# OpenGene/gencore

Measured on AMD Instinct MI355X. Metric: consensus read-pairs/sec (whole node) + clustering HBM GB/s vs roofline, higher is better.
Workload: dtype u8

## Files before the change

### gencore_amd/capi.py

```python
import ctypes as C
import os

import numpy as np

GCE_ABI_VERSION = 3
GCE_NONE = 0xFFFFFFFF
GCE_MAX_SUPPORTING_READS = 100
UINT64_MAX = 0xFFFFFFFFFFFFFFFF

_HERE = os.path.dirname(os.path.abspath(__file__))
LIB_PATH = os.path.join(_HERE, "csrc", "libgencore_amd.so")

CORE_DTYPE = np.dtype(
    [("tid", "<i4"), ("pos", "<i4"), ("l_qname", "u1"), ("mapq", "u1"), ("bin", "<u2"), ("n_cigar", "<u2"),
     ("flag", "<u2"), ("l_qseq", "<i4"), ("mtid", "<i4"), ("mpos", "<i4"), ("isize", "<i4")])
assert CORE_DTYPE.itemsize == 32


class GceParams(C.Structure):
    _fields_ = [
        ("abi_version", C.c_int32), ("device", C.c_int32),
        ("proper_umi_diff_threshold", C.c_int32), ("unproper_umi_diff_threshold", C.c_int32),
        ("duplex_mismatch_threshold", C.c_int32), ("cluster_size_req", C.c_int32),
        ("base_score_req", C.c_int32), ("high_quality", C.c_int32), ("moderate_quality", C.c_int32),
        ("low_quality", C.c_int32), ("score_high", C.c_int32), ("score_moderate", C.c_int32),
        ("score_low", C.c_int32), ("score_bad", C.c_int32),
        ("skip_low_complexity_cluster_threshold", C.c_int32), ("duplex_only", C.c_int32),
        ("disable_duplex", C.c_int32), ("flush_period", C.c_int32),
        ("score_percent_req", C.c_double), ("umi_prefix", C.c_char * 32),
        ("n_targets", C.c_int32), ("target_len", C.c_void_p),
        ("tick_offset", C.c_int64), ("trailing_flush", C.c_int32), ("max_contig", C.c_int32),
    ]


class GceBatch(C.Structure):
    _fields_ = [
        ("n_reads", C.c_int64), ("core", C.c_void_p),
        ("qname_off", C.c_void_p), ("qname", C.c_void_p),
        ("cigar_off", C.c_void_p), ("cigar", C.c_void_p),
        ("seq_off", C.c_void_p), ("seq", C.c_void_p),
        ("qual_off", C.c_void_p), ("qual", C.c_void_p),
        ("nm", C.c_void_p), ("nm_type", C.c_void_p),
        ("mi_off", C.c_void_p), ("mi", C.c_void_p),
        ("qname_bytes", C.c_size_t), ("cigar_words", C.c_size_t), ("seq_bytes", C.c_size_t),
        ("qual_bytes", C.c_size_t), ("mi_bytes", C.c_size_t),
        ("tick", C.c_void_p),
    ]


class GceStats(C.Structure):
    _fields_ = [(n, C.c_int64) for n in (
        "reads", "bases", "reads_unmapped", "bases_unmapped", "base_mismatches", "reads_with_mismatches",
        "clusters", "multi_molecule_clusters", "molecules", "molecules_se", "molecules_pe", "sscs", "dcs",
        "uncounted_supporting_reads")] + [("supporting_hist", C.c_int64 * GCE_MAX_SUPPORTING_READS)]

    def as_dict(self):
        d = {n: int(getattr(self, n)) for n, _ in self._fields_[:-1]}
        d["supporting_hist"] = [int(x) for x in self.supporting_hist]
        return d

    def as_array(self):
        return np.frombuffer(bytes(self), dtype=np.int64).copy()


GCE_STATS_WORDS = 14 + GCE_MAX_SUPPORTING_READS
assert C.sizeof(GceStats) == 8 * GCE_STATS_WORDS


class GceResult(C.Structure):
    _fields_ = [
        ("n_reads", C.c_int64), ("n_out", C.c_int64), ("src", C.c_void_p), ("kind", C.c_void_p), ("qname_src", C.c_void_p),
        ("nm_new", C.c_void_p), ("fr", C.c_void_p), ("rr", C.c_void_p), ("mate", C.c_void_p), ("seq_off", C.c_void_p),
        ("qual_off", C.c_void_p), ("seq", C.c_void_p), ("qual", C.c_void_p), ("seq_bytes", C.c_size_t), ("qual_bytes", C.c_size_t),
        ("pre", GceStats), ("post", GceStats),
    ]


class GceTiming(C.Structure):
    _fields_ = [(n, C.c_double) for n in (
        "total_ms", "describe_ms", "cluster_ms", "csr_ms", "pairing_ms", "score_ms", "consensus_ms", "finish_ms", "output_ms")] + [
        ("n_clusters", C.c_int64), ("n_groups", C.c_int64), ("n_pairs", C.c_int64), ("n_leaders", C.c_int64)]

    def as_dict(self):
        return {n: getattr(self, n) for n, _ in self._fields_}


STATUS_NAMES = {
    0: "GCE_OK", -1: "GCE_ERR_INVALID", -2: "GCE_ERR_NO_DEVICE", -3: "GCE_ERR_HIP", -4: "GCE_ERR_OOM",
    -10: "GCE_ERR_UNSORTED", -11: "GCE_ERR_UMI_MISMATCH", -12: "GCE_ERR_NM_MISSING", -13: "GCE_ERR_UMI_PARSE",
    -14: "GCE_ERR_QNAME_SHORT", -15: "GCE_ERR_REF_WINDOW"}

EXPORTED_SYMBOLS = [
    "gce_params_default", "gce_detect_umi_prefix", "gce_create", "gce_destroy", "gce_set_reference", "gce_set_reference_ascii", "gce_set_reference_window",
    "gce_pack_reference", "gce_set_flush_events", "gce_submit", "gce_submit_device", "gce_process", "gce_drain", "gce_result_device",
    "gce_get_timing", "gce_get_vote_counters", "gce_get_consensus_counters", "gce_get_skipped_groups", "gce_get_index_counters", "gce_get_pairing_tiers", "gce_reset", "gce_last_error", "gce_status_message", "gce_abi_version",
    "gce_reserve", "gce_submit_async", "gce_submit_wait",
    "gce_bam_open", "gce_bam_close", "gce_bam_error", "gce_bam_get_info", "gce_bam_chunk", "gce_bam_write", "gce_bam_from_batch", "gce_sam_to_bam", "gce_bam_to_sam",
    "gce_fasta_load", "gce_fasta_get", "gce_fasta_free", "gce_run_bam", "gce_run_bam_hostcodec", "gce_run_bam_sharded", "gce_run_bam_sharded_hostcodec", "gce_raw_deflate_output", "gce_raw_read_deflated_async", "gce_bgzf_deflate", "gce_raw_deflate_output_codes", "gce_bgzf_deflate_codes", "gce_raw_attach_mirror", "gce_raw_select_shard", "gce_raw_merge_outputs", "gce_raw_begin", "gce_raw_push", "gce_raw_push_bgzf", "gce_bgzf_inflate", "gce_raw_finish", "gce_raw_build_output", "gce_raw_read_output_async", "gce_host_alloc", "gce_host_free", "gce_depth_stats", "gce_stats_payload_device", "gce_stats_payload_sum", "gce_stats_payload_read", "gce_run_bam_depth", "gce_depth_run_free", "gce_stats_device", "gce_stream_context", "gce_plan_shards", "gce_free", "gce_bed_load", "gce_bed_free",
    "gce_report_json", "gce_report_summary", "gce_bam_read_header", "gce_bam_header_free", "gce_run_bam_passes", "gce_device_bytes", "gce_bam_index", "gce_bam_sort", "gce_bam_sort_passes", "gce_sam_parse", "gce_sam_sort",
    "gce_sam_format", "gce_raw_format_output", "gce_raw_read_text_async", "gce_get_sam_format_counters",
    "gce_bam_calmd"]


class GceBamInfo(C.Structure):
    _fields_ = [("n_targets", C.c_int32), ("target_len", C.POINTER(C.c_uint32)), ("target_name", C.POINTER(C.c_char_p)),
                ("text", C.c_void_p), ("l_text", C.c_int64), ("n_records", C.c_int64),
                ("qname_bytes", C.c_uint64), ("cigar_words", C.c_uint64), ("seq_bytes", C.c_uint64), ("qual_bytes", C.c_uint64),
                ("mi_bytes", C.c_uint64), ("read_s", C.c_double), ("inflate_s", C.c_double), ("index_s", C.c_double)]


class GceDepth(C.Structure):
    _fields_ = [("n_targets", C.c_int32), ("bin_off", C.POINTER(C.c_int64)), ("pre_depth", C.POINTER(C.c_int64)), ("post_depth", C.POINTER(C.c_int64)),
                ("n_regions", C.c_int32), ("pre_bed", C.POINTER(C.c_int64)), ("post_bed", C.POINTER(C.c_int64))]


class GcePayloadLayout(C.Structure):
    _fields_ = [("stats_words", C.c_int32), ("n_targets", C.c_int32), ("n_bins", C.c_int64), ("n_regions", C.c_int32), ("total_words", C.c_int64),
                ("bin_off", C.POINTER(C.c_int64))]


class GceDepthRun(C.Structure):
    _fields_ = [("n_targets", C.c_int32), ("n_bins", C.c_int64), ("bin_off", C.POINTER(C.c_int64)), ("pre_depth", C.POINTER(C.c_int64)), ("post_depth", C.POINTER(C.c_int64)),
                ("n_regions", C.c_int32), ("region_tid", C.POINTER(C.c_int32)), ("region_start", C.POINTER(C.c_int32)), ("region_end", C.POINTER(C.c_int32)),
                ("pre_bed", C.POINTER(C.c_int64)), ("post_bed", C.POINTER(C.c_int64)), ("pre", GceStats), ("post", GceStats), ("payload_bytes", C.c_int64)]


class GcePassRun(C.Structure):
    _fields_ = [("n_passes", C.c_int32), ("single_pass", C.c_int32), ("reads_per_pass", C.c_int64 * 64), ("held_max", C.c_int64), ("peak_device_bytes", C.c_int64),
                ("budget_bytes", C.c_int64),
                ("fixed_bytes", C.c_int64), ("pass_room", C.c_int64), ("total_weight", C.c_int64), ("key_pass_s", C.c_double), ("pass_s", C.c_double * 64)]


class GceBaiRun(C.Structure):
    _fields_ = [("n_records", C.c_int64), ("n_no_coor", C.c_int64), ("n_bins", C.c_int64), ("n_chunks", C.c_int64), ("n_intervals", C.c_int64),
                ("n_ref", C.c_int32), ("pad", C.c_int32), ("read_s", C.c_double), ("gpu_s", C.c_double), ("write_s", C.c_double), ("total_s", C.c_double)]


class GceSortRun(C.Structure):
    _fields_ = [("n_records", C.c_int64), ("n_no_coor", C.c_int64), ("n_descents", C.c_int64), ("inflated_bytes", C.c_int64), ("out_bytes", C.c_int64),
                ("peak_device_bytes", C.c_int64), ("n_ref", C.c_int32), ("pad", C.c_int32), ("read_s", C.c_double), ("inflate_index_s", C.c_double),
                ("sort_s", C.c_double), ("gather_s", C.c_double), ("write_s", C.c_double), ("total_s", C.c_double)]


class GceCalmdRun(C.Structure):
    _fields_ = [("n_records", C.c_int64), ("n_rewritten", C.c_int64), ("n_unchanged", C.c_int64), ("n_no_ref", C.c_int64), ("n_nm_changed", C.c_int64),
                ("n_md_changed", C.c_int64), ("inflated_bytes", C.c_int64), ("out_record_bytes", C.c_int64), ("out_bytes", C.c_int64), ("peak_device_bytes", C.c_int64),
                ("n_ref", C.c_int32), ("pad", C.c_int32), ("read_s", C.c_double), ("inflate_index_s", C.c_double), ("calmd_s", C.c_double), ("write_s", C.c_double),
                ("total_s", C.c_double)]


class GceSortPassRun(C.Structure):
    _fields_ = [("n_passes", C.c_int32), ("in_core", C.c_int32), ("pass_bytes", C.c_int64), ("resident_bytes", C.c_int64), ("key_pass_s", C.c_double),
                ("plan_s", C.c_double), ("pass_s", C.c_double * 64)]


class GceBamRun(C.Structure):
    _fields_ = [("n_reads", C.c_int64), ("n_out", C.c_int64), ("open_s", C.c_double), ("read_s", C.c_double), ("inflate_s", C.c_double), ("index_s", C.c_double), ("submit_s", C.c_double),
                ("process_s", C.c_double), ("kernel_ms", C.c_double), ("drain_s", C.c_double), ("write_s", C.c_double),
                ("total_s", C.c_double), ("pre", GceStats), ("post", GceStats), ("peak_rss_kb", C.c_int64), ("rss_start_kb", C.c_int64), ("rss_end_kb", C.c_int64)]


class GceError(RuntimeError):
    def __init__(self, status, detail=""):
        self.status = status
        super().__init__("%s (%d): %s" % (STATUS_NAMES.get(status, "?"), status, detail))


_lib = None


def load_library(path=None, mode=C.RTLD_GLOBAL):
    global _lib
    if _lib is not None and path is None:
        return _lib
    p = path or os.environ.get("GCE_LIB") or LIB_PATH
    if not os.path.exists(p):
        raise OSError("libgencore_amd.so not built at %s — run `python -c 'import __graft_entry__ as g; g.build()'`" % p)
    lib = C.CDLL(p, mode=mode)
    lib.gce_params_default.argtypes = [C.POINTER(GceParams)]
    lib.gce_params_default.restype = None
    lib.gce_detect_umi_prefix.argtypes = [C.c_char_p, C.c_char * 32]
    lib.gce_detect_umi_prefix.restype = None
    lib.gce_create.argtypes = [C.POINTER(GceParams), C.POINTER(C.c_void_p)]
    lib.gce_destroy.argtypes = [C.c_void_p]
    lib.gce_destroy.restype = None
    lib.gce_set_reference.argtypes = [C.c_void_p, C.c_int32, C.c_void_p, C.c_int64]
    lib.gce_set_reference_ascii.argtypes = [C.c_void_p, C.c_int32, C.c_void_p, C.c_int64]
    lib.gce_set_reference_window.argtypes = [C.c_void_p, C.c_int32, C.c_int64, C.c_int64, C.c_void_p, C.c_int64]
    lib.gce_pack_reference.argtypes = [C.c_char_p, C.c_int64, C.c_void_p]
    lib.gce_pack_reference.restype = None
    lib.gce_set_flush_events.argtypes = [C.c_void_p, C.c_int32, C.c_void_p, C.c_void_p]
    lib.gce_submit.argtypes = [C.c_void_p, C.POINTER(GceBatch)]
    lib.gce_submit_device.argtypes = [C.c_void_p, C.POINTER(GceBatch)]
    lib.gce_process.argtypes = [C.c_void_p]
    lib.gce_drain.argtypes = [C.c_void_p, C.POINTER(GceResult)]
    lib.gce_result_device.argtypes = [C.c_void_p, C.POINTER(GceResult)]
    lib.gce_get_timing.argtypes = [C.c_void_p, C.POINTER(GceTiming)]
    lib.gce_get_vote_counters.argtypes = [C.c_void_p, C.POINTER(C.c_int64)]
    lib.gce_get_consensus_counters.argtypes = [C.c_void_p, C.POINTER(C.c_int64)]
    lib.gce_get_skipped_groups.argtypes = [C.c_void_p, C.POINTER(C.c_int64)]
    lib.gce_get_index_counters.argtypes = [C.c_void_p, C.POINTER(C.c_int64)]
    lib.gce_get_pairing_tiers.argtypes = [C.c_void_p, C.c_int64, C.c_void_p, C.c_void_p, C.POINTER(C.c_int64), C.POINTER(C.c_int64)]
    lib.gce_stats_device.argtypes = [C.c_void_p, C.POINTER(C.c_void_p)]
    lib.gce_stream_context.argtypes = [C.c_int32, C.c_void_p, C.c_int64, C.c_int32, C.c_void_p, C.POINTER(C.c_int32), C.POINTER(C.POINTER(C.c_int32)), C.POINTER(C.POINTER(C.c_int32))]
    lib.gce_plan_shards.argtypes = [C.c_int32, C.c_void_p, C.c_int64, C.c_int32, C.c_int32, C.c_void_p]
    lib.gce_free.argtypes = [C.c_void_p]
    lib.gce_free.restype = None
    lib.gce_reset.argtypes = [C.c_void_p]
    lib.gce_last_error.argtypes = [C.c_void_p]
    lib.gce_last_error.restype = C.c_char_p
    lib.gce_status_message.argtypes = [C.c_int]
    lib.gce_status_message.restype = C.c_char_p
    lib.gce_abi_version.restype = C.c_int
    lib.gce_reserve.argtypes = [C.c_void_p, C.c_int64, C.c_size_t, C.c_size_t, C.c_size_t, C.c_size_t]
    lib.gce_submit_async.argtypes = [C.c_void_p, C.POINTER(GceBatch), C.POINTER(C.c_int32)]
    lib.gce_submit_wait.argtypes = [C.c_void_p, C.c_int32]
    lib.gce_bam_open.argtypes = [C.c_char_p, C.c_int, C.POINTER(C.c_void_p)]
    lib.gce_bam_close.argtypes = [C.c_void_p]
    lib.gce_bam_close.restype = None
    lib.gce_bam_error.argtypes = [C.c_void_p]
    lib.gce_bam_error.restype = C.c_char_p
    lib.gce_bam_get_info.argtypes = [C.c_void_p, C.POINTER(GceBamInfo)]
    lib.gce_bam_chunk.argtypes = [C.c_void_p, C.c_int64, C.c_int64, C.c_int, C.POINTER(GceBatch)]
    lib.gce_bam_write.argtypes = [C.c_char_p, C.c_void_p, C.POINTER(GceResult), C.c_int, C.c_int]
    lib.gce_bam_from_batch.argtypes = [C.c_char_p, C.POINTER(GceBatch), C.c_int32, C.c_void_p, C.POINTER(C.c_char_p), C.c_char_p, C.c_int, C.c_int]
    lib.gce_sam_to_bam.argtypes = [C.c_char_p, C.c_char_p, C.c_int, C.c_int, C.c_char_p]
    lib.gce_bam_to_sam.argtypes = [C.c_char_p, C.c_char_p, C.c_int, C.c_char_p]
    lib.gce_fasta_load.argtypes = [C.c_char_p, C.c_int, C.POINTER(C.c_void_p)]
    lib.gce_fasta_get.argtypes = [C.c_void_p, C.POINTER(C.c_int32), C.POINTER(C.POINTER(C.c_char_p)), C.POINTER(C.POINTER(C.c_void_p)), C.POINTER(C.POINTER(C.c_int64))]
    lib.gce_fasta_free.argtypes = [C.c_void_p]
    lib.gce_fasta_free.restype = None
    lib.gce_depth_stats.argtypes = [C.c_void_p, C.c_int32, C.c_int32, C.c_void_p, C.c_void_p, C.c_void_p, C.POINTER(GceDepth)]
    lib.gce_stats_payload_device.argtypes = [C.c_void_p, C.c_int32, C.c_int32, C.c_void_p, C.c_void_p, C.c_void_p, C.POINTER(C.c_void_p), C.POINTER(GcePayloadLayout)]
    lib.gce_stats_payload_sum.argtypes = [C.POINTER(C.c_void_p), C.c_int32, C.POINTER(C.c_void_p), C.POINTER(GcePayloadLayout)]
    lib.gce_stats_payload_read.argtypes = [C.c_void_p, C.c_void_p, C.c_int64, C.c_void_p]
    lib.gce_run_bam_depth.argtypes = [C.c_char_p, C.c_char_p, C.c_char_p, C.c_char_p, C.c_int32, C.POINTER(GceParams), C.c_int32, C.c_void_p, C.c_int32, C.c_int, C.c_int,
                                      C.POINTER(GceBamRun), C.POINTER(GceDepthRun), C.c_char_p]
    lib.gce_run_bam_passes.argtypes = [C.c_char_p, C.c_char_p, C.c_char_p, C.c_char_p, C.c_int32, C.POINTER(GceParams), C.c_int32, C.c_int, C.c_int, C.c_size_t, C.c_int32, C.c_size_t,
                                       C.POINTER(GceBamRun), C.POINTER(GceDepthRun), C.POINTER(GcePassRun), C.c_char_p]
    lib.gce_device_bytes.argtypes = [C.POINTER(C.c_int64), C.POINTER(C.c_int64), C.c_int32]
    lib.gce_bam_index.argtypes = [C.c_char_p, C.c_char_p, C.c_int32, C.c_int, C.c_uint64, C.POINTER(GceBaiRun), C.c_char_p]
    if hasattr(lib, "gce_bam_sort"):
        lib.gce_bam_sort.argtypes = [C.c_char_p, C.c_char_p, C.c_int32, C.c_int, C.c_int, C.c_uint64, C.c_size_t, C.POINTER(GceSortRun), C.c_char_p]
    if hasattr(lib, "gce_bam_sort_passes"):
        lib.gce_bam_sort_passes.argtypes = [C.c_char_p, C.c_char_p, C.c_int32, C.c_int, C.c_int, C.c_uint64, C.c_size_t, C.c_int32, C.POINTER(GceSortRun),
                                            C.POINTER(GceSortPassRun), C.c_char_p]
    if hasattr(lib, "gce_sam_parse"):
        lib.gce_sam_parse.argtypes = [C.c_int32, C.c_char_p, C.c_size_t, C.c_int32, C.POINTER(C.c_char_p), C.c_void_p, C.c_size_t, C.POINTER(C.c_size_t), C.POINTER(C.c_int64),
                                      C.POINTER(C.c_int64), C.POINTER(C.c_int64), C.c_char_p]
    if hasattr(lib, "gce_sam_sort"):
        lib.gce_sam_sort.argtypes = [C.c_char_p, C.c_char_p, C.c_int32, C.c_int, C.c_int, C.c_uint64, C.c_size_t, C.POINTER(GceSortRun), C.POINTER(C.c_int64), C.c_char_p]
    if hasattr(lib, "gce_sam_format"):
        lib.gce_sam_format.argtypes = [C.c_int32, C.c_void_p, C.c_size_t, C.c_int32, C.POINTER(C.c_char_p), C.c_void_p, C.c_size_t, C.POINTER(C.c_size_t), C.POINTER(C.c_int64),
                                       C.POINTER(C.c_int64), C.POINTER(C.c_int64), C.c_char_p]
        lib.gce_raw_format_output.argtypes = [C.c_void_p, C.c_int32, C.POINTER(C.c_char_p), C.POINTER(C.c_uint64)]
        lib.gce_raw_read_text_async.argtypes = [C.c_void_p, C.c_uint64, C.c_void_p, C.c_size_t, C.POINTER(C.c_int32)]
        lib.gce_get_sam_format_counters.argtypes = [C.POINTER(C.c_int64)]
    if hasattr(lib, "gce_bam_calmd"):
        lib.gce_bam_calmd.argtypes = [C.c_char_p, C.c_char_p, C.c_char_p, C.c_int32, C.c_int, C.c_int, C.c_uint64, C.c_size_t, C.POINTER(GceCalmdRun), C.c_char_p]
    lib.gce_depth_run_free.argtypes = [C.POINTER(GceDepthRun)]
    lib.gce_depth_run_free.restype = None
    lib.gce_bed_load.argtypes = [C.c_char_p, C.c_int32, C.POINTER(C.c_char_p), C.POINTER(C.c_int32), C.POINTER(C.POINTER(C.c_int32)), C.POINTER(C.POINTER(C.c_int32)),
                                 C.POINTER(C.POINTER(C.c_int32)), C.POINTER(C.POINTER(C.c_char_p))]
    lib.gce_bed_free.argtypes = [C.c_int32, C.c_void_p, C.c_void_p, C.c_void_p, C.c_void_p]
    lib.gce_bed_free.restype = None
    lib.gce_report_json.argtypes = [C.c_char_p, C.POINTER(GceStats), C.POINTER(GceStats), C.POINTER(GceDepthRun), C.POINTER(C.c_char_p), C.POINTER(C.c_char_p),
                                    C.c_int32, C.c_int32, C.c_char_p, C.c_char * 256]
    lib.gce_report_summary.argtypes = [C.POINTER(GceStats), C.c_int32, C.c_char_p, C.c_size_t, C.POINTER(C.c_size_t)]
    lib.gce_bam_read_header.argtypes = [C.c_char_p, C.POINTER(C.c_int32), C.POINTER(C.POINTER(C.c_char_p)), C.POINTER(C.POINTER(C.c_uint32)), C.c_char * 256]
    lib.gce_bam_header_free.argtypes = [C.c_int32, C.POINTER(C.c_char_p), C.POINTER(C.c_uint32)]
    lib.gce_bam_header_free.restype = None
    lib.gce_bgzf_inflate.argtypes = [C.c_int32, C.c_void_p, C.c_size_t, C.c_int32, C.c_void_p, C.c_void_p, C.c_void_p, C.c_void_p, C.POINTER(C.c_int32)]
    lib.gce_bgzf_deflate.argtypes = [C.c_int32, C.c_void_p, C.c_size_t, C.c_uint32, C.c_void_p, C.c_size_t, C.POINTER(C.c_size_t)]
    if hasattr(lib, "gce_bgzf_deflate_codes"):
        lib.gce_bgzf_deflate_codes.argtypes = [C.c_int32, C.c_void_p, C.c_size_t, C.c_uint32, C.c_int32, C.c_void_p, C.c_size_t, C.POINTER(C.c_size_t)]
        lib.gce_raw_deflate_output_codes.argtypes = [C.c_void_p, C.c_int32, C.POINTER(C.c_uint64)]
    lib.gce_run_bam_sharded.argtypes = [C.c_char_p, C.c_char_p, C.c_char_p, C.POINTER(GceParams), C.c_int32, C.POINTER(C.c_int32), C.c_int32, C.c_int, C.c_int, C.POINTER(GceBamRun), C.c_char * 256]
    lib.gce_run_bam.argtypes = [C.c_char_p, C.c_char_p, C.c_char_p, C.POINTER(GceParams), C.c_int, C.c_int64, C.c_int, C.POINTER(GceBamRun), C.c_char * 256]
    if path is None:
        _lib = lib
    return lib


def default_params(lib=None, **overrides):
    p = GceParams()
# ... 25 lines not shown
```

### gencore_amd/csrc/engine.hip

```cpp
#include <hip/hip_runtime.h>
#include <hip/hip_ext.h>
#include <cstdio>
#include <cstdlib>
#include <algorithm>
#include <cstring>
#include <ctime>
#include <string>
#include <vector>

#include "gce_kernels.hpp"
#include "gce_pair2.hpp"
#include "gce_vote.hpp"
#include "gce_deep.hpp"
#include "gce_output.hpp"
#include "gce_depth.hpp"
#include "gce_inflate.hpp"
#include "gce_deflate.hpp"

namespace {

static thread_local double t_alloc_s = 0.0; static thread_local long t_alloc_n = 0; static thread_local size_t t_alloc_bytes = 0;
static inline double mono_s() { struct timespec ts; clock_gettime(CLOCK_MONOTONIC, &ts); return (double)ts.tv_sec + 1e-9 * (double)ts.tv_nsec; }
long long g_dev_live = 0, g_dev_peak = 0;
static int64_t g_pass_idx_ctr[4] = {0, 0, 0, 0};
inline void dev_bytes_add(long long d) {
    const long long now = __atomic_add_fetch(&g_dev_live, d, __ATOMIC_RELAXED);
    long long pk = __atomic_load_n(&g_dev_peak, __ATOMIC_RELAXED);
    while (now > pk && !__atomic_compare_exchange_n(&g_dev_peak, &pk, now, true, __ATOMIC_RELAXED, __ATOMIC_RELAXED)) {}
}
struct DevBuf {
    void *p = nullptr; size_t cap = 0;
    static size_t padded(size_t bytes) { return bytes + bytes / 8 + 256; }
    hipError_t ensure(size_t bytes) { return bytes <= cap && p ? hipSuccess : take(padded(bytes)); }
    hipError_t take(size_t want) {
        const double t0 = mono_s();
        release();
        hipError_t e = hipMalloc(&p, want);
        if (e == hipSuccess) { cap = want; dev_bytes_add((long long)want); } else p = nullptr;
        t_alloc_s += mono_s() - t0; t_alloc_n++; t_alloc_bytes += want;
        return e;
    }
    void release() { if (p) { (void)hipFree(p); dev_bytes_add(-(long long)cap); } p = nullptr; cap = 0; }
    template <class T> T *as() const { return (T *)p; }
};
struct ScopedBuf : DevBuf { ~ScopedBuf() { release(); } };

enum { EV_START = 0, EV_CLUSTER, EV_CSR, EV_DESCRIBE, EV_PAIRING, EV_SCORE, EV_CONSENSUS, EV_FINISH, EV_OUTPUT, EV_COUNT };

}

#include "gce_devstream.hpp"

struct HostRaw {
    uint8_t *p = nullptr; size_t n = 0, cap = 0;
    ~HostRaw() { free(p); }
    void resize(size_t k) { if (k > cap) { free(p); p = (uint8_t *)malloc(k ? k : 1); cap = p ? k : 0; } n = p ? k : 0; }
    uint8_t *data() { return p; }
    size_t size() const { return n; }
    bool empty() const { return n == 0; }
};

struct gce_engine {
    gce_params prm{};
    bool vote_off_logged = false;
    std::vector<uint32_t> target_len;
    std::string err;
    hipStream_t stream = nullptr;
    hipEvent_t ev[EV_COUNT]{};
    std::vector<DevBuf> ref_buf; std::vector<const uint8_t *> ref_ptr; std::vector<int64_t> ref_len, ref_win; bool have_win = false;
    DevBuf d_ref_ptr, d_ref_len, d_ref_win, d_target_len, d_target_cum;
    std::vector<const uint8_t *> up_ref_ptr; std::vector<int64_t> up_ref_len, up_win; std::vector<uint32_t> up_tl; const void *up_dev[5]{}; bool up_valid = false;
    std::vector<gce_core> h_core; std::vector<uint64_t> h_qoff, h_coff, h_soff, h_loff, h_mioff;
    std::vector<char> h_qname, h_mi; std::vector<uint32_t> h_cigar; std::vector<uint8_t> h_seq, h_qual, h_nmt; std::vector<int32_t> h_nm; std::vector<uint64_t> h_tick;
    std::vector<int32_t> h_ev_tid, h_ev_pos;
    bool have_mi = false, have_tick = false, have_events = false, host_mode = false, device_mode = false, processed = false;
    bool reserved = false; hipStream_t up_stream = nullptr; std::vector<hipEvent_t> up_events;
    hipStream_t aux_stream = nullptr; hipEvent_t aux_ev[4]{};
    size_t rs_n = 0, rs_q = 0, rs_c = 0, rs_s = 0, rs_l = 0, st_n = 0, st_q = 0, st_c = 0, st_s = 0, st_l = 0, st_m = 0; bool dev_concat = false;
    gce_batch dev_batch{};
    DevBuf b_core, b_qoff, b_qname, b_coff, b_cigar, b_soff, b_seq, b_loff, b_qual, b_nm, b_nmt, b_mioff, b_mi, b_tick;
    DevBuf uinfo, rdesc, spatch, slot, score, out_flag, orec, out_index, nmx;
    DevBuf o_src, o_kind, o_qsrc, o_nm, o_fr, o_rr, o_mate, o_soff, o_qoff, o_seq, o_qual, o_key, o_rec, o_ksoff, o_kqoff, o_krow, o_rank64, o_part3, ref_ascii;
    int64_t n_out = 0; size_t out_seq_bytes = 0, out_qual_bytes = 0; int dev_error = 0; uint32_t dev_error_read = 0;
    DevBuf lrec, lout, bhdr, blk_base, ev_tid, ev_pos, ev_read, table, toff;
    DevBuf raw, rw_tmp, rw_ncig, rw_nmpos, rw_rsize, rw_roff, rw_body; RecIdx rw;
    size_t raw_n = 0; bool raw_mode = false; int64_t raw_records = 0; uint64_t raw_body_bytes = 0;
    int64_t idx_ctr[4] = {0, 0, 0, 0};
    DevBuf z_comp, z_dir, z_err; size_t z_n = 0; std::vector<InfDir> z_members;
    DevBuf zo_slots, zo_sizes, zo_off, zo_out; uint64_t zo_bytes = 0;
    DevBuf sf_text; uint64_t sf_bytes = 0; int64_t raw_body_nrec = -1;
    std::vector<gce_engine *> mirrors;
    DevBuf sh_tickall, sh_shard, sh_flag, sh_sel, sh_core, sh_qoff, sh_coff, sh_soff, sh_loff, sh_nm, sh_nmt, sh_mioff, sh_tick, sh_roff, sh_nmpos, sh_keys, sh_stage; int64_t shard_n = -1;
    bool shard_cut_done = false;
    bool tab_clean = false; const void *tab_clean_ptr = nullptr; size_t tab_clean_cap = 0;
    DevBuf cl_ikey, cl_start, cl_n, cl_npairs, cl_ngroups, cl_gbase, cl_nresult, cl_hasumi, cl_tier;
    DevBuf members, sorted, pl, pr, pu, pg, gpl, gpr, grp_begin, grp_n, gl_cluster, g_begin, g_np;
    DevBuf slow_args, deep_list, k64, slow_list, left_list, pf_flag, pf_list, pq_flag, pq_list, p16_flag, p16_list, pd_slab, gen_flag, gen_list, score_list, gw, vlive, vb_start, rp_left, rp_right, rp_merge, rp_rmerge, rp_umi, rp_umilen, rp_state, rp_supp, rp_nm, rp_qsl, rp_qsr, scan_part, si;
    StreamInfo h_si{};
    void *si_pin = nullptr, *si_pin_dev = nullptr; unsigned long long si_seq = 0;
    gce_timing timing{};
    int64_t n = 0, n_pre = 0;
    DevBuf dp_binoff, dp_regoff, dp_rs, dp_re, dp_pmax, dp_sorted, dp_depth, dp_bed, dp_where;
    std::vector<int64_t> h_binoff, h_depth_pre, h_depth_post, h_bed_pre, h_bed_post; int64_t payload_words = 0;
    std::vector<uint8_t> r_kind; HostRaw r_seq, r_qual; std::vector<uint32_t> r_src, r_qsrc, r_mate; std::vector<int32_t> r_nm; std::vector<int16_t> r_fr, r_rr;
    std::vector<uint64_t> r_soff, r_qoff;
};

static int fail(gce_engine *e, int code, const std::string &msg) { if (e) e->err = msg; return code; }
#define HIPCHK(call) do { hipError_t _e = (call); if (_e != hipSuccess) return fail(e, _e == hipErrorOutOfMemory ? GCE_ERR_OOM : GCE_ERR_HIP, std::string(#call) + ": " + hipGetErrorString(_e)); } while (0)

extern "C" {

int gce_abi_version(void) { return GCE_ABI_VERSION; }

void gce_params_default(gce_params *p) {
    memset(p, 0, sizeof *p);
    p->abi_version = GCE_ABI_VERSION;
    p->proper_umi_diff_threshold = 1; p->unproper_umi_diff_threshold = 0; p->duplex_mismatch_threshold = 2;
    p->cluster_size_req = 1; p->base_score_req = 6; p->high_quality = 30; p->moderate_quality = 20; p->low_quality = 15;
    p->score_high = 8; p->score_moderate = 6; p->score_low = 4; p->score_bad = 2;
    p->skip_low_complexity_cluster_threshold = 1000; p->flush_period = 10000; p->score_percent_req = 0.8;
}

void gce_detect_umi_prefix(const char *q, char out[32]) {
    memset(out, 0, 32);
    if (strstr(q, "umi_")) strcpy(out, "umi");
    else if (strstr(q, "UMI_")) strcpy(out, "UMI");
}

const char *gce_status_message(int s) {
    switch (s) {
    case GCE_OK: return "ok";
    case GCE_ERR_INVALID: return "invalid argument or call order";
    case GCE_ERR_NO_DEVICE: return "no HIP device available (this engine has no CPU fallback)";
    case GCE_ERR_HIP: return "HIP runtime error";
    case GCE_ERR_OOM: return "out of device memory";
    case GCE_ERR_UNSORTED: return "ERROR: the input is unsorted. Please sort the input first.";
    case GCE_ERR_UMI_MISMATCH: return "The UMI of a read pair should be identical";
    case GCE_ERR_NM_MISSING: return "NM tag missing on a consensus template whose mismatch count changed";
    case GCE_ERR_UMI_PARSE: return "UMI parse: substr start beyond the end of the read name";
    case GCE_ERR_QNAME_SHORT: return "copyQName ERROR: desitination qname is shorter";
    case GCE_ERR_REF_WINDOW: return "reference window: a clustered read lies outside the bases staged for its contig";
    default: return "unknown status";
    }
}

const char *gce_last_error(const gce_engine *e) { return e ? e->err.c_str() : "null engine"; }

int gce_create(const gce_params *params, gce_engine **out) {
    if (!params || !out || params->abi_version != GCE_ABI_VERSION) return GCE_ERR_INVALID;
    if (params->proper_umi_diff_threshold < 0 || params->unproper_umi_diff_threshold < 0 || params->flush_period < 0) return GCE_ERR_INVALID;
    int ndev = 0;
    if (hipGetDeviceCount(&ndev) != hipSuccess || ndev <= 0 || params->device >= ndev) return GCE_ERR_NO_DEVICE;
    gce_engine *e = new gce_engine();
    e->prm = *params;
    if (e->prm.flush_period == 0) e->prm.flush_period = 10000;
    if (params->n_targets > 0 && params->target_len) e->target_len.assign(params->target_len, params->target_len + params->n_targets);
    e->prm.target_len = nullptr;
    if (hipSetDevice(params->device) != hipSuccess || hipStreamCreate(&e->stream) != hipSuccess) { delete e; return GCE_ERR_HIP; }
    for (auto &v : e->ev) (void)hipEventCreate(&v);
    *out = e;
    return GCE_OK;
}

void gce_destroy(gce_engine *e) {
    if (!e) return;
    (void)hipSetDevice(e->prm.device);
    (void)hipStreamSynchronize(e->stream);
    DevBuf *all[] = {&e->d_ref_ptr, &e->d_ref_len, &e->d_ref_win, &e->d_target_len, &e->d_target_cum, &e->b_core, &e->b_qoff, &e->b_qname, &e->b_coff, &e->b_cigar, &e->b_soff,
                     &e->b_seq, &e->b_loff, &e->b_qual, &e->b_nm, &e->b_nmt, &e->b_mioff, &e->b_mi, &e->b_tick, &e->uinfo, &e->rdesc, &e->spatch,
                     &e->slot, &e->score, &e->out_flag, &e->orec, &e->out_index, &e->nmx, &e->o_src, &e->o_kind, &e->o_qsrc, &e->o_nm, &e->o_fr, &e->o_rr, &e->o_mate,
                     &e->o_key, &e->o_rec, &e->o_ksoff, &e->o_kqoff, &e->o_krow, &e->o_rank64, &e->o_part3, &e->o_soff, &e->o_qoff, &e->o_seq, &e->o_qual, &e->ref_ascii, &e->lrec, &e->lout, &e->bhdr,
                     &e->blk_base, &e->ev_tid, &e->ev_pos, &e->ev_read, &e->table, &e->toff, &e->cl_ikey, &e->cl_start, &e->cl_n,
                     &e->cl_npairs, &e->cl_ngroups, &e->cl_gbase, &e->cl_nresult, &e->cl_hasumi, &e->cl_tier, &e->members, &e->sorted, &e->pl, &e->pr, &e->pu,
                     &e->pg, &e->gpl, &e->gpr, &e->grp_begin, &e->grp_n, &e->gl_cluster, &e->g_begin, &e->g_np, &e->deep_list, &e->k64, &e->slow_list, &e->pf_flag, &e->pf_list, &e->pq_flag, &e->pq_list, &e->left_list, &e->slow_args, &e->pd_slab, &e->gen_flag, &e->gen_list, &e->score_list, &e->gw, &e->vlive, &e->vb_start, &e->rp_left, &e->rp_right, &e->rp_merge, &e->rp_rmerge,
                     &e->rp_umi, &e->rp_umilen, &e->rp_state, &e->rp_supp, &e->rp_nm, &e->rp_qsl, &e->rp_qsr, &e->scan_part, &e->si};
    for (auto *b : all) b->release();
    for (DevBuf *b : {&e->z_comp, &e->z_dir, &e->z_err, &e->raw, &e->rw_tmp, &e->rw_ncig, &e->rw_nmpos, &e->rw_rsize, &e->rw_roff, &e->rw_body, &e->sf_text}) b->release();
    e->rw.release();
    for (DevBuf *b : {&e->zo_slots, &e->zo_sizes, &e->zo_off, &e->zo_out, &e->p16_flag, &e->p16_list}) b->release();
    for (DevBuf *b : {&e->sh_tickall, &e->sh_shard, &e->sh_flag, &e->sh_sel, &e->sh_core, &e->sh_qoff, &e->sh_coff, &e->sh_soff, &e->sh_loff, &e->sh_nm, &e->sh_nmt, &e->sh_mioff, &e->sh_tick, &e->sh_roff, &e->sh_nmpos, &e->sh_keys, &e->sh_stage}) b->release();
    for (DevBuf *b : {&e->dp_binoff, &e->dp_regoff, &e->dp_rs, &e->dp_re, &e->dp_pmax, &e->dp_sorted, &e->dp_depth, &e->dp_bed, &e->dp_where}) b->release();
    for (auto ev : e->up_events) (void)hipEventDestroy(ev);
    if (e->up_stream) { (void)hipStreamSynchronize(e->up_stream); (void)hipStreamDestroy(e->up_stream); }
    if (e->aux_stream) { (void)hipStreamSynchronize(e->aux_stream); (void)hipStreamDestroy(e->aux_stream); }
    for (auto &v : e->aux_ev) if (v) (void)hipEventDestroy(v);
    for (auto &b : e->ref_buf) b.release();
    for (auto &v : e->ev) if (v) (void)hipEventDestroy(v);
    if (e->stream) (void)hipStreamDestroy(e->stream);
    if (e->si_pin) (void)hipHostFree(e->si_pin);
    delete e;
}

void gce_pack_reference(const char *bases, int64_t n, uint8_t *out) {
    memset(out, 0, (size_t)((n + 1) / 2));
    for (int64_t i = 0; i < n; i++) {
        uint8_t code;
        switch (bases[i]) { case 'A': code = 1; break; case 'T': code = 2; break; case 'C': code = 3; break; case 'G': code = 4; break; default: code = 0; }
        out[i >> 1] |= (i & 1) ? (uint8_t)(code << 4) : code;
    }
}

int gce_set_reference(gce_engine *e, int32_t tid, const uint8_t *nibbles, int64_t n_bases) {
    if (!e || tid < 0 || n_bases < 0) return GCE_ERR_INVALID;
    (void)hipSetDevice(e->prm.device);
    if ((size_t)tid >= e->ref_buf.size()) { e->ref_buf.resize(tid + 1); e->ref_ptr.resize(tid + 1, nullptr); e->ref_len.resize(tid + 1, 0); }
    if (!nibbles) { e->ref_ptr[tid] = nullptr; e->ref_len[tid] = 0; return GCE_OK; }
    size_t bytes = (size_t)((n_bases + 1) / 2);
    HIPCHK(e->ref_buf[tid].ensure(bytes + 16));
    hipPointerAttribute_t attr; bool is_dev = hipPointerGetAttributes(&attr, nibbles) == hipSuccess && attr.type == hipMemoryTypeDevice;
    (void)hipGetLastError();
    HIPCHK(hipMemcpyAsync(e->ref_buf[tid].p, nibbles, bytes, is_dev ? hipMemcpyDeviceToDevice : hipMemcpyHostToDevice, e->stream));
    HIPCHK(hipStreamSynchronize(e->stream));
    e->ref_ptr[tid] = e->ref_buf[tid].as<uint8_t>(); e->ref_len[tid] = n_bases;
    if (2 * (size_t)tid + 1 < e->ref_win.size()) e->ref_win[2 * tid] = e->ref_win[2 * tid + 1] = 0;
    return GCE_OK;
}

int gce_set_reference_ascii(gce_engine *e, int32_t tid, const char *bases, int64_t n_bases) {
    if (!e || tid < 0 || n_bases < 0 || (!bases && n_bases > 0)) return GCE_ERR_INVALID;
    (void)hipSetDevice(e->prm.device);
    if ((size_t)tid >= e->ref_buf.size()) { e->ref_buf.resize(tid + 1); e->ref_ptr.resize(tid + 1, nullptr); e->ref_len.resize(tid + 1, 0); }
    const size_t bytes = (size_t)((n_bases + 1) / 2);
    HIPCHK(e->ref_buf[tid].ensure(bytes + 16));
    HIPCHK(e->ref_ascii.ensure((size_t)n_bases + 16));
    hipPointerAttribute_t attr; const bool is_dev = hipPointerGetAttributes(&attr, bases) == hipSuccess && attr.type == hipMemoryTypeDevice;
    (void)hipGetLastError();
    if (n_bases) {
        HIPCHK(hipMemcpyAsync(e->ref_ascii.p, bases, (size_t)n_bases, is_dev ? hipMemcpyDeviceToDevice : hipMemcpyHostToDevice, e->stream));
        const unsigned grid = (unsigned)std::min<uint64_t>((bytes + 255) / 256, 65535u * 4u);
        hipLaunchKernelGGL(k_pack_reference, dim3(grid), dim3(256), 0, e->stream, (const char *)e->ref_ascii.p, n_bases, e->ref_buf[tid].as<uint8_t>());
    }
    HIPCHK(hipStreamSynchronize(e->stream));
    HIPCHK(hipGetLastError());
    e->ref_ptr[tid] = e->ref_buf[tid].as<uint8_t>(); e->ref_len[tid] = n_bases;
    if (2 * (size_t)tid + 1 < e->ref_win.size()) e->ref_win[2 * tid] = e->ref_win[2 * tid + 1] = 0;
    return GCE_OK;
}

int gce_set_reference_window(gce_engine *e, int32_t tid, int64_t contig_len, int64_t win_start, const char *bases, int64_t n_bases) {
    if (!e || tid < 0 || contig_len < 0 || win_start < 0 || (win_start & 1) || n_bases < 0 || win_start + n_bases > contig_len || (!bases && n_bases > 0)) return GCE_ERR_INVALID;
    const int rc = gce_set_reference_ascii(e, tid, bases, n_bases);
    if (rc != GCE_OK) return rc;
    if (e->ref_win.size() < 2 * e->ref_ptr.size()) e->ref_win.resize(2 * e->ref_ptr.size(), 0);
    e->ref_ptr[tid] = e->ref_buf[tid].as<uint8_t>() - (win_start >> 1);
    e->ref_len[tid] = contig_len;
    e->ref_win[2 * tid] = win_start; e->ref_win[2 * tid + 1] = win_start + n_bases;
    e->have_win = true;
    return GCE_OK;
}

int gce_reset(gce_engine *e) {
    if (!e) return GCE_ERR_INVALID;
    e->h_core.clear(); e->h_qoff.clear(); e->h_coff.clear(); e->h_soff.clear(); e->h_loff.clear(); e->h_mioff.clear(); e->h_tick.clear();
    e->h_qname.clear(); e->h_mi.clear(); e->h_cigar.clear(); e->h_seq.clear(); e->h_qual.clear(); e->h_nmt.clear(); e->h_nm.clear();
    e->have_mi = e->have_tick = e->host_mode = e->device_mode = e->processed = e->raw_mode = false; e->n = 0; e->n_out = 0; e->shard_n = -1; e->shard_cut_done = false;
    e->st_n = e->st_q = e->st_c = e->st_s = e->st_l = e->st_m = 0; e->dev_concat = false;
    return GCE_OK;
}

int gce_set_flush_events(gce_engine *e, int32_t n_events, const int32_t *ev_tid, const int32_t *ev_pos) {
    if (!e || n_events < 0 || (n_events > 0 && (!ev_tid || !ev_pos))) return GCE_ERR_INVALID;
    e->h_ev_tid.assign(ev_tid, ev_tid + n_events); e->h_ev_pos.assign(ev_pos, ev_pos + n_events);
// ... 396 lines not shown
    const bool same = e->up_valid && e->up_ref_ptr == e->ref_ptr && e->up_ref_len == e->ref_len && e->up_tl == e->target_len && e->up_win == win && memcmp(dev_now, e->up_dev, sizeof dev_now) == 0;
    if (!same) {
        e->up_valid = false;
        if (nref) {
            HIPCHK(hipMemcpyAsync(e->d_ref_ptr.p, e->ref_ptr.data(), (size_t)nref * 8, hipMemcpyHostToDevice, e->stream));
            HIPCHK(hipMemcpyAsync(e->d_ref_len.p, e->ref_len.data(), (size_t)nref * 8, hipMemcpyHostToDevice, e->stream));
        }
        std::vector<uint64_t> cum(e->target_len.size()); uint64_t acc = 0;
        for (size_t i = 0; i < cum.size(); i++) { cum[i] = acc; acc += e->target_len[i]; }
        if (!e->target_len.empty()) {
            HIPCHK(hipMemcpyAsync(e->d_target_len.p, e->target_len.data(), e->target_len.size() * 4, hipMemcpyHostToDevice, e->stream));
            HIPCHK(hipMemcpyAsync(e->d_target_cum.p, cum.data(), cum.size() * 8, hipMemcpyHostToDevice, e->stream));
        }
        if (!win.empty()) HIPCHK(hipMemcpyAsync(e->d_ref_win.p, win.data(), win.size() * 8, hipMemcpyHostToDevice, e->stream));
        HIPCHK(hipStreamSynchronize(e->stream));
        e->up_ref_ptr = e->ref_ptr; e->up_ref_len = e->ref_len; e->up_tl = e->target_len; e->up_win = win; memcpy(e->up_dev, dev_now, sizeof dev_now);
        e->up_valid = true;
    }
    DevParams p{};
    p.proper_thr = e->prm.proper_umi_diff_threshold; p.unproper_thr = e->prm.unproper_umi_diff_threshold;
    p.duplex_mismatch_thr = e->prm.duplex_mismatch_threshold; p.cluster_size_req = e->prm.cluster_size_req; p.base_score_req = e->prm.base_score_req;
    p.high_q = e->prm.high_quality; p.moderate_q = e->prm.moderate_quality; p.low_q = e->prm.low_quality;
    p.s_high = e->prm.score_high; p.s_moderate = e->prm.score_moderate; p.s_low = e->prm.score_low; p.s_bad = e->prm.score_bad;
    p.skip_low_complexity_thr = e->prm.skip_low_complexity_cluster_threshold; p.duplex_only = e->prm.duplex_only; p.disable_duplex = e->prm.disable_duplex;
    p.period = e->prm.flush_period; p.score_percent_req = e->prm.score_percent_req;
    {
        int mn = std::min(std::min(p.s_high, p.s_moderate), std::min(p.s_low, p.s_bad)), mx = std::max(std::max(p.s_high, p.s_moderate), std::max(p.s_low, p.s_bad));
        p.score_bias = std::max(0, 3 - mn); p.score_max = std::max(0, mx + 4);
        if (p.score_max + p.score_bias > 255) return fail(e, GCE_ERR_INVALID, "score constants out of range");
        auto by = [&](int sc) { return (uint32_t)((sc + p.score_bias) & 0xFF); };
        p.q2s_lut = by(p.s_bad) | by(p.s_low) << 8 | by(p.s_moderate) << 16 | by(p.s_high) << 24;
        p.thr_low4 = 0x01010101u * (uint32_t)(p.low_q & 0xFF); p.thr_mod4 = 0x01010101u * (uint32_t)(p.moderate_q & 0xFF); p.thr_high4 = 0x01010101u * (uint32_t)(p.high_q & 0xFF);
        p.q2s_swar_ok = p.low_q >= 0 && p.low_q <= p.moderate_q && p.moderate_q <= p.high_q && p.high_q <= 127;
        p.s_min_lb = mn;
        p.vote_ok = mn >= 0 && mx + 4 <= 120 && p.moderate_q >= 0 && p.moderate_q <= 127 && p.base_score_req <= 100 && p.q2s_swar_ok;
        p.vote_accept_by_qual = std::min(std::min(p.s_moderate, p.s_high), mn + 4) >= std::max(p.base_score_req, 1);
        if (!p.vote_ok && !e->vote_off_logged) {
            e->vote_off_logged = true;
            const char *why = !p.q2s_swar_ok ? "quality thresholds not nested (low <= moderate <= high <= 127)" : mn < 0 ? "a score constant below 0"
                            : mx + 4 > 120 ? "a score constant above 116" : (p.moderate_q < 0 || p.moderate_q > 127) ? "moderate quality outside 0..127" : "base_score_req above 100";
            fprintf(stderr, "gencore_amd: k_vote off for this engine (%s): every group goes to the per-side kernels\n", why);
        }
    }
    memcpy(p.prefix, e->prm.umi_prefix, 32); p.prefix[31] = 0; p.prefix_len = (int)strlen(p.prefix);
    p.n_targets = (int)e->target_len.size(); p.target_len = e->d_target_len.as<uint32_t>(); p.target_cum = e->target_len.empty() ? nullptr : e->d_target_cum.as<uint64_t>();
    p.tick_offset = e->have_tick ? 0 : e->prm.tick_offset; p.tick_epoch0 = p.tick_offset / p.period; p.tick_rem0 = (int32_t)(p.tick_offset % p.period); p.trailing_flush = e->have_tick ? 0 : e->prm.trailing_flush;
    {
        uint32_t mx = 1; for (uint32_t v : e->target_len) mx = std::max(mx, v);
        int bt = 1; while (bt < 31 && (1ll << bt) < (long long)std::max<size_t>(e->target_len.size(), 1)) bt++;
        int bl = 1; while (bl < 32 && (1ull << bl) <= (uint64_t)mx) bl++;
        p.key_bt = bt; p.key_bl = bl;
    }
    p.n_ref = nref; p.ref_data = e->d_ref_ptr.as<const uint8_t *>(); p.ref_len = e->d_ref_len.as<int64_t>(); p.ref_win = win.empty() ? nullptr : e->d_ref_win.as<int64_t>();

    Work w{};
    const int64_t n_sblk = (N + SB_READS - 1) / SB_READS;
    w.n_sblk = n_sblk;
    const int64_t max_events = e->have_tick ? (int64_t)e->h_ev_tid.size() + 2 : (p.tick_offset % p.period + N) / p.period + 2;
    w.max_events = (int)max_events;
    uint64_t T = ((uint64_t)n1 + (uint64_t)n1 / 4 + 2 * SCAN_TILE - 1) / SCAN_TILE * SCAN_TILE;
    w.tsize = T; w.tinv = 1.0 / (double)T;
    {
        uint64_t genome = 0; for (uint32_t v : e->target_len) genome += v;
        const uint64_t qmax = (genome * TAB_WAYS + TAB_WAYS) / T + 1;
        int cb = 1; while (cb < 33 && (1ull << cb) <= (uint64_t)N + 1024) cb++;
        int qb = 1; while (qb < 52 && (1ull << qb) <= qmax) qb++;
        p.nw_cb = cb; p.nw_bd = 62 - cb - qb; p.nw_ok = !e->target_len.empty() && p.nw_bd >= 1;
        if (p.nw_bd > 40) p.nw_bd = 40;
    }
    const size_t qual_bytes = hb.qual_bytes ? hb.qual_bytes : 1;
    const size_t nsb1 = (size_t)(n_sblk > 0 ? n_sblk : 1);
#define ENS(buf, bytes) HIPCHK(e->buf.ensure(bytes))
    ENS(uinfo, n1 * 8); ENS(rdesc, n1 * sizeof(ReadDescP)); ENS(spatch, n1 * 4); ENS(slot, n1 * 4 + 16); ENS(score, qual_bytes + 64);
    ENS(out_flag, n1 + 144);        ENS(nmx, n1 * 4); ENS(orec, n1 * sizeof(OutRec)); ENS(out_index, n1 * 4);
    ENS(lrec, nsb1 * SB_READS * sizeof(LeadRec)); ENS(lout, nsb1 * SB_READS * sizeof(LeadOut));
    ENS(bhdr, nsb1 * sizeof(BlkHdr)); ENS(blk_base, nsb1 * 4);
    ENS(ev_tid, (size_t)max_events * 4); ENS(ev_pos, (size_t)max_events * 4); ENS(ev_read, (size_t)max_events * 4);
    ENS(table, T * sizeof(TabEntry)); ENS(toff, T * 4);
    ENS(k64, n1 * 24); ENS(members, n1 * 4); ENS(sorted, n1 * 4); ENS(pl, n1 * 4); ENS(pr, n1 * 4); ENS(pu, n1 * 4); ENS(pg, n1 * 4); ENS(gpl, n1 * 4); ENS(gpr, n1 * 4);
    ENS(grp_begin, n1 * 4); ENS(grp_n, n1 * 4); ENS(slow_list, n1 * 4 + 64);
    w.slow_list = e->slow_list.as<uint32_t>();
    ENS(deep_list, (n1 / 64 + 64) * 16); w.deep_list = e->deep_list.p;
    const unsigned nblk_N = cdiv(n1, SCAN_TILE);
    ENS(scan_part, std::max<size_t>(2 * nsb1, (size_t)2 * nblk_N) * 8 + 16);     ENS(si, sizeof(StreamInfo));
    w.uinfo = e->uinfo.as<uint64_t>(); w.rdesc = e->rdesc.as<ReadDescP>(); w.spatch = e->spatch.as<uint32_t>();
    w.slot = e->slot.as<uint32_t>(); w.score = e->score.as<int8_t>();
    w.out_flag = e->out_flag.as<uint8_t>(); w.nmx = e->nmx.as<uint32_t>(); w.orec = e->orec.as<OutRec>(); w.out_index = e->out_index.as<uint32_t>();
    w.lrec = e->lrec.as<LeadRec>(); w.lout = e->lout.as<LeadOut>(); w.bhdr = e->bhdr.as<BlkHdr>(); w.blk_base = e->blk_base.as<uint32_t>();
    w.ev_tid = e->ev_tid.as<int32_t>(); w.ev_pos = e->ev_pos.as<int32_t>(); w.ev_read = e->ev_read.as<uint32_t>();
    w.tab = e->table.as<TabEntry>(); w.toff = e->toff.as<uint32_t>();
    w.k64 = e->k64.as<uint64_t>(); w.members = e->members.as<uint32_t>(); w.sorted = e->sorted.as<uint32_t>(); w.pl = e->pl.as<uint32_t>(); w.pr = e->pr.as<uint32_t>();
    w.pu = e->pu.as<uint32_t>(); w.pg = e->pg.as<uint32_t>(); w.gpl = e->gpl.as<uint32_t>(); w.gpr = e->gpr.as<uint32_t>();
    w.grp_begin = e->grp_begin.as<uint32_t>(); w.grp_n = e->grp_n.as<uint32_t>();
    w.scan_part = e->scan_part.as<uint64_t>(); w.si = e->si.as<StreamInfo>();
    ENS(cl_ikey, n1 * 4); ENS(cl_start, n1 * 4); ENS(cl_n, n1 * 4);
    w.cl_ikey = e->cl_ikey.as<uint32_t>(); w.cl_start = e->cl_start.as<uint32_t>(); w.cl_n = e->cl_n.as<uint32_t>();

    StreamInfo init{}; init.first_unmapped = NONE32; init.err_key = ~0ull; init.lq_min = 0x7FFFFFFF; init.lq_max = -1;
    if (e->have_tick) { init.n_events = init.n_events_a = (int)e->h_ev_tid.size(); }
    HIPCHK(hipMemcpyAsync(e->si.p, &init, sizeof init, hipMemcpyHostToDevice, e->stream));
    if (e->have_tick && !e->h_ev_tid.empty()) {
        HIPCHK(hipMemcpyAsync(e->ev_tid.p, e->h_ev_tid.data(), e->h_ev_tid.size() * 4, hipMemcpyHostToDevice, e->stream));
        HIPCHK(hipMemcpyAsync(e->ev_pos.p, e->h_ev_pos.data(), e->h_ev_pos.size() * 4, hipMemcpyHostToDevice, e->stream));
    }
    hipStream_t s = e->stream;
    if (!e->tab_clean || e->tab_clean_ptr != e->table.p || e->tab_clean_cap != e->table.cap) {
        HIPCHK(hipMemsetAsync(e->table.p, 0, e->table.cap, s));
        e->tab_clean_ptr = e->table.p; e->tab_clean_cap = e->table.cap;
    }
    e->tab_clean = false;
    HIPCHK(hipEventRecord(e->ev[EV_START], s));
    HIPCHK(hipMemsetAsync(e->out_flag.p, 0, n1, s));
    if (N > 0) LAUNCH_EV(k_cluster, dim3((unsigned)n_sblk), dim3(SB_T), s, e->ev[EV_CLUSTER], b, p, w);
#ifdef CL_PROF
    if (N > 0) {
        StreamInfo hs; (void)hipStreamSynchronize(s); (void)hipMemcpy(&hs, e->si.p, sizeof hs, hipMemcpyDeviceToHost);
        static const char *nm[3] = {"key records + keys", "LDS leaders", "stores"};
        const double blocks = (double)hs.prof[15];
        fprintf(stderr, "k_cluster phases, mean per block (us), %.0f blocks:", blocks);
        for (int k = 0; k < 3; k++) fprintf(stderr, " %s %.2f;", nm[k], blocks ? hs.prof[k] / blocks / 100.0 : 0.0);
        fprintf(stderr, "\n");
    }
#endif
    if (N <= 0) HIPCHK(hipEventRecord(e->ev[EV_CLUSTER], s));
    CANARY("EV_CLUSTER");
    if (N > 0) {
        if (!e->have_tick) {
            hipLaunchKernelGGL(k_blk_scan, dim3(1), dim3(1024), 0, s, w, p);
            hipLaunchKernelGGL(k_events, dim3(cdiv(max_events, EV_T / 64)), dim3(EV_T), 0, s, b, p, w);
        }
        const unsigned nb4 = cdiv(n_sblk, 4);
        hipLaunchKernelGGL(k_leaders, dim3(nb4), dim3(256), 0, s, b, p, w);
        hipLaunchKernelGGL(k_num_reduce, dim3(nb4), dim3(256), 0, s, w, p.nw_cb);
        hipLaunchKernelGGL(k_scan_partials, dim3(1), dim3(1024), 0, s, w.scan_part, (uint64_t)nb4, &w.si->n_clusters, (unsigned long long *)nullptr);
        hipLaunchKernelGGL(k_num_apply, dim3(nb4), dim3(256), 0, s, w);
        LAUNCH_EV(k_scatter, dim3((unsigned)n_sblk), dim3(SB_T), s, e->ev[EV_CSR], N, w);
    } else HIPCHK(hipEventRecord(e->ev[EV_CSR], s));
    CANARY("EV_CSR");
    unsigned long long si_seq1 = 0;
    if ((rc = read_si_begin(e, &si_seq1)) != GCE_OK) return rc;
    if (N > 0) {
#ifndef GCE_DESCRIBE_BLOCKS
#define GCE_DESCRIBE_BLOCKS 32768
#endif
        const int64_t n_tiles = (N + 255) / 256;
        int tpb = (int)((n_tiles + GCE_DESCRIBE_BLOCKS - 1) / GCE_DESCRIBE_BLOCKS); if (tpb < 1) tpb = 1;
        LAUNCH_EV(k_describe, dim3(cdiv(n_tiles, tpb)), dim3(256), s, e->ev[EV_DESCRIBE], b, p, w, tpb);
    } else HIPCHK(hipEventRecord(e->ev[EV_DESCRIBE], s));
    CANARY("EV_DESCRIBE");
    if ((rc = read_si_end(e, si_seq1)) != GCE_OK) return rc;
    HIPCHK(hipGetLastError());
    e->tab_clean = true;
    const uint32_t C = (uint32_t)e->h_si.n_clusters;
    const size_t c1 = C ? C : 1;
    ENS(cl_npairs, c1 * 4); ENS(cl_ngroups, c1 * 4); ENS(cl_gbase, c1 * 4); ENS(cl_nresult, c1 * 4); ENS(cl_hasumi, c1); ENS(cl_tier, c1);
    w.cl_npairs = e->cl_npairs.as<uint32_t>(); w.cl_ngroups = e->cl_ngroups.as<uint32_t>(); w.cl_gbase = e->cl_gbase.as<uint32_t>();
    w.cl_nresult = e->cl_nresult.as<uint32_t>(); w.cl_hasumi = e->cl_hasumi.as<uint8_t>(); w.cl_tier = e->cl_tier.as<uint8_t>();
    uint32_t NG = 0;
    bool si_behind_describe = false;
    if (C > 0 && e->dev_error == 0) {
        ENS(left_list, c1 * 4 + 64); w.left_list = e->left_list.as<uint32_t>();
        ENS(pf_flag, c1 + 64); ENS(pf_list, c1 * 4); ENS(pq_flag, c1 + 64); ENS(pq_list, c1 * 4); ENS(p16_flag, c1 + 64); ENS(p16_list, c1 * 4);
        w.pf_flag = e->pf_flag.as<uint8_t>(); w.pf_list = e->pf_list.as<uint32_t>(); w.pq_flag = e->pq_flag.as<uint8_t>(); w.pq_list = e->pq_list.as<uint32_t>(); w.p16_flag = e->p16_flag.as<uint8_t>(); w.p16_list = e->p16_list.as<uint32_t>();
        const bool pair_classes = (double)N > 10.0 * (double)C;
        if (!pair_classes) fill_many(s, {FillSeg{e->pf_flag.p, c1, 0u, 0u}, FillSeg{e->pq_flag.p, c1, 0u, 0u}});
        const unsigned nbc = cdiv(C, SCAN_TILE);
        auto compact = [&](uint8_t *flag, uint32_t *list, unsigned long long *count) {
            hipLaunchKernelGGL(k_flag_reduce, dim3(nbc), dim3(256), 0, s, (const uint8_t *)flag, (uint64_t)C, w.scan_part);
            hipLaunchKernelGGL(k_scan_partials, dim3(1), dim3(1024), 0, s, w.scan_part, (uint64_t)nbc, count, (unsigned long long *)nullptr);
            hipLaunchKernelGGL(k_flag_apply, dim3(nbc), dim3(256), 0, s, (const uint8_t *)flag, (uint64_t)C, (const uint64_t *)w.scan_part, list);
        };
#ifdef PS_STOP
        {
            hipEvent_t a_, b_, c_; (void)hipEventCreate(&a_); (void)hipEventCreate(&b_); (void)hipEventCreate(&c_);
            (void)hipEventRecord(a_, s);
            hipLaunchKernelGGL(k_pairing_sub<16>, dim3(cdiv(C, 4 * WAVES_PER_BLOCK)), dim3(256), 0, s, b, p, w, C, (const uint32_t *)nullptr, (const unsigned long long *)nullptr, w.pq_flag, 0);
            (void)hipEventRecord(b_, s);
            hipLaunchKernelGGL(k_pairing_sub<32>, dim3(cdiv(C, 2 * WAVES_PER_BLOCK)), dim3(256), 0, s, b, p, w, C, (const uint32_t *)nullptr, (const unsigned long long *)nullptr, w.pf_flag, 0);
            (void)hipEventRecord(c_, s); (void)hipEventSynchronize(c_);
            float m1 = 0, m2 = 0; (void)hipEventElapsedTime(&m1, a_, b_); (void)hipEventElapsedTime(&m2, b_, c_);
            fprintf(stderr, "k_pairing_sub up to tick %d: <16> %.3f ms, <32> over ALL clusters %.3f ms\n", PS_STOP, m1, m2);
            return fail(e, GCE_ERR_INVALID, "experiment build");
        }
#endif
        ENS(pd_slab, PD_BIG_BLOCKS * PD_SLAB);
        if (pair_classes) {
            hipLaunchKernelGGL(k_pair_class_reduce, dim3(nbc), dim3(256), 0, s, (const uint32_t *)w.cl_n, C, w.scan_part);
            hipLaunchKernelGGL(k_scan_partials, dim3(1), dim3(1024), 0, s, w.scan_part, (uint64_t)nbc, &w.si->n_p16_items, &w.si->n_pq_items);
            hipLaunchKernelGGL(k_pair_class_apply, dim3(nbc), dim3(256), 0, s, (const uint32_t *)w.cl_n, C, (const uint64_t *)w.scan_part, w.p16_list, w.pq_list, w.pf_list, w.si);
            static const bool tiers_aux = getenv("GCE_NO_AUX_STREAM") == nullptr;
            hipStream_t s2 = s;
            if (tiers_aux) {
                if ((rc = aux_ready(e)) != GCE_OK) return rc;
                s2 = e->aux_stream;
                HIPCHK(hipEventRecord(e->aux_ev[0], s));
                HIPCHK(hipStreamWaitEvent(s2, e->aux_ev[0], 0));
            }
            hipLaunchKernelGGL(k_pairing_fast, dim3(2048), dim3(256), 0, s2, b, p, w, C, (const uint32_t *)w.pf_list);
            hipLaunchKernelGGL(k_pairing_deep<false>, dim3(256), dim3(PD_T), 0, s2, b, p, w, (uint8_t *)nullptr);
            if (tiers_aux) HIPCHK(hipEventRecord(e->aux_ev[1], s2));
            hipLaunchKernelGGL(k_pairing_sub<16>, dim3(cdiv(C, 4 * WAVES_PER_BLOCK)), dim3(256), 0, s, b, p, w, C, (const uint32_t *)w.p16_list, (const unsigned long long *)&w.si->n_p16_items, w.pq_flag, 1);
            hipLaunchKernelGGL(k_pairing_sub<32>, dim3(cdiv(C, 2 * WAVES_PER_BLOCK)), dim3(256), 0, s, b, p, w, C, (const uint32_t *)w.pq_list, (const unsigned long long *)&w.si->n_pq_items, w.pf_flag, 1);
            if (tiers_aux) HIPCHK(hipStreamWaitEvent(s, e->aux_ev[1], 0));
        } else {
            hipLaunchKernelGGL(k_pairing_sub<16>, dim3(cdiv(C, 4 * WAVES_PER_BLOCK)), dim3(256), 0, s, b, p, w, C, (const uint32_t *)nullptr, (const unsigned long long *)nullptr, w.pq_flag, 0);
            compact(w.pq_flag, w.pq_list, &w.si->n_pq_items);
            hipLaunchKernelGGL(k_pairing_sub<32>, dim3(cdiv(C, 2 * WAVES_PER_BLOCK)), dim3(256), 0, s, b, p, w, C, (const uint32_t *)w.pq_list, (const unsigned long long *)&w.si->n_pq_items, w.pf_flag, 0);
            compact(w.pf_flag, w.pf_list, &w.si->n_pf_items);
            hipLaunchKernelGGL(k_pairing_fast, dim3(2048), dim3(256), 0, s, b, p, w, C, (const uint32_t *)w.pf_list);
            hipLaunchKernelGGL(k_pairing_deep<false>, dim3(256), dim3(PD_T), 0, s, b, p, w, (uint8_t *)nullptr);
        }
        hipLaunchKernelGGL(k_pairing_deep<true>, dim3(PD_BIG_BLOCKS), dim3(PD_T), 0, s, b, p, w, e->pd_slab.as<uint8_t>());
        hipLaunchKernelGGL(k_pairing_slow<0>, dim3(1024), dim3(256), 0, s, b, p, w);
        hipLaunchKernelGGL(k_pairing_slow<1>, dim3(1024, 16), dim3(256), 0, s, b, p, w);
        hipLaunchKernelGGL(k_pairing_slow<2>, dim3(1024), dim3(256), 0, s, b, p, w);
        const unsigned nblk_C = cdiv(C, SCAN_TILE);
        hipLaunchKernelGGL(k_scan_reduce, dim3(nblk_C), dim3(256), 0, s, (const uint32_t *)w.cl_ngroups, (uint64_t)C, w.scan_part);
        hipLaunchKernelGGL(k_scan_partials, dim3(1), dim3(1024), 0, s, w.scan_part, (uint64_t)nblk_C, &w.si->n_pairs , &w.si->n_groups);
        hipLaunchKernelGGL(k_u32_apply, dim3(nblk_C), dim3(256), 0, s, (const uint32_t *)w.cl_ngroups, w.cl_gbase, (uint64_t)C, (const uint64_t *)w.scan_part);
        ENS(gl_cluster, n1 * 4); ENS(g_begin, n1 * 4); ENS(g_np, n1 * 4); ENS(gw, n1 * 8); ENS(vlive, n1 * 16);
        const size_t vb_cap = ((VB_MINW + 3) * n1) / VB_W + 8;
        ENS(vb_start, vb_cap * 4);
        w.gl_cluster = e->gl_cluster.as<uint32_t>(); w.g_begin = e->g_begin.as<uint32_t>(); w.g_np = e->g_np.as<uint32_t>();
        w.gw = e->gw.as<uint64_t>(); w.vlive = e->vlive.as<uint4>(); w.vb_start = e->vb_start.as<uint32_t>();
        HIPCHK(hipMemsetAsync(e->vb_start.p, 0xFF, vb_cap * 4, s));
        hipLaunchKernelGGL(k_group_fill, dim3(cdiv(C, 256)), dim3(256), 0, s, p, w, C, (uint32_t)VB_W, (uint32_t)VB_MINW);
        hipLaunchKernelGGL(k_u64_reduce, dim3(nblk_N), dim3(256), 0, s, (const uint64_t *)w.gw, (const unsigned long long *)&w.si->n_groups, w.scan_part);
        hipLaunchKernelGGL(k_u64_partials, dim3(1), dim3(1024), 0, s, w.scan_part, (const unsigned long long *)&w.si->n_groups, &w.si->vote_weight, &w.si->n_live);
        LAUNCH_EV(k_vote_batches, dim3(nblk_N), dim3(256), s, e->ev[EV_PAIRING], w, (const unsigned long long *)&w.si->n_groups, (const uint64_t *)w.scan_part);
        CANARY("EV_PAIRING");
        if ((rc = read_si(e)) != GCE_OK) return rc;
        HIPCHK(hipGetLastError());
        si_behind_describe = true;
        NG = (uint32_t)e->h_si.n_groups;
    } else HIPCHK(hipEventRecord(e->ev[EV_PAIRING], s));
    const size_t g1 = NG ? NG : 1;
    ENS(gen_list, g1 * 8); ENS(gen_flag, g1 * 2 + 64); ENS(score_list, n1 * 4 + 64);       ENS(rp_left, g1 * 4); ENS(rp_right, g1 * 4); ENS(rp_merge, g1 * 4); ENS(rp_rmerge, g1 * 4); ENS(rp_umi, g1 * 8);
    ENS(rp_umilen, g1 * 2); ENS(rp_state, g1); ENS(rp_supp, g1 * 4); ENS(rp_nm, g1 * 8); ENS(rp_qsl, g1 * 4); ENS(rp_qsr, g1 * 4);
    w.gen_list = e->gen_list.as<uint32_t>(); w.gen_flag = e->gen_flag.as<uint8_t>(); w.score_list = e->score_list.as<uint32_t>();
    w.rp_left = e->rp_left.as<uint32_t>(); w.rp_right = e->rp_right.as<uint32_t>();
    w.rp_merge = e->rp_merge.as<uint32_t>(); w.rp_rmerge = e->rp_rmerge.as<uint32_t>(); w.rp_umi = e->rp_umi.as<const char *>();
    w.rp_umilen = e->rp_umilen.as<uint16_t>(); w.rp_state = e->rp_state.as<uint8_t>(); w.rp_supp = e->rp_supp.as<int32_t>();
    w.rp_nm = e->rp_nm.as<int32_t>(); w.rp_qsl = e->rp_qsl.as<uint32_t>(); w.rp_qsr = e->rp_qsr.as<uint32_t>();
    if (NG > 0 && e->dev_error == 0) {
        {
            SlowArgs sa; sa.b = b; sa.p = p; sa.w = w;
            HIPCHK(e->slow_args.ensure(sizeof sa));
            HIPCHK(hipMemcpyAsync(e->slow_args.p, &sa, sizeof sa, hipMemcpyHostToDevice, s));
        }
        fill_many(s, {FillSeg{e->gen_flag.p, g1 * 2, 0u, 0u},
                      FillSeg{e->rp_nm.p, g1 * 8, 0xFFu, 0u},
                      FillSeg{e->rp_left.p, g1 * 4, 0xFFu, 0u}, FillSeg{e->rp_right.p, g1 * 4, 0xFFu, 0u}});
        const uint32_t n_live = (uint32_t)e->h_si.n_live;
#ifdef VB_XCD
        const unsigned nbatch = (((unsigned)(e->h_si.vote_weight / VB_W) + 1u) + 7u) & ~7u;
#else
        const unsigned nbatch = (unsigned)(e->h_si.vote_weight / VB_W) + 1u;
#endif
#ifdef VB_STOP
        {
            hipEvent_t a_, b_; (void)hipEventCreate(&a_); (void)hipEventCreate(&b_);
            (void)hipEventRecord(a_, s); hipLaunchKernelGGL(k_vote, dim3(nbatch), dim3(VB_T), 0, s, b, p, w, n_live); (void)hipEventRecord(b_, s); (void)hipEventSynchronize(b_);
            float ms_ = 0; (void)hipEventElapsedTime(&ms_, a_, b_); fprintf(stderr, "k_vote up to tick %d: %.3f ms\n", VB_STOP, ms_);
            return fail(e, GCE_ERR_INVALID, "experiment build");
        }
#endif
        LAUNCH_EV(k_vote, dim3(nbatch), dim3(VB_T), s, e->ev[EV_SCORE], b, p, w, n_live);
        CANARY("EV_SCORE");
        const bool deep_stream = ((double)N > 48.0 * (double)NG || getenv("GCE_FORCE_AUX_STREAM")) && !getenv("GCE_NO_AUX_STREAM");
        const unsigned cf_cap = deep_stream ? 32768u : 4096u, sc2_cap = deep_stream ? 16384u : 2048u;
        const unsigned cf_grid = std::min<unsigned>(cdiv(2ull * NG, WAVES_PER_BLOCK), cf_cap);
        const unsigned sc2_grid = std::min<unsigned>(cdiv(N, 2 * WAVES_PER_BLOCK * 64), sc2_cap);
        if (deep_stream) {
            if ((rc = aux_ready(e)) != GCE_OK) return rc;
            HIPCHK(hipEventRecord(e->aux_ev[0], s));
            HIPCHK(hipStreamWaitEvent(e->aux_stream, e->aux_ev[0], 0));
            hipLaunchKernelGGL(k_score2, dim3(sc2_grid), dim3(256), 0, e->aux_stream, b, p, w);
            HIPCHK(hipEventRecord(e->aux_ev[1], e->aux_stream));
            hipLaunchKernelGGL(k_deep_prepare, dim3(1024), dim3(256), 0, s, b, p, w);
            HIPCHK(hipStreamWaitEvent(s, e->aux_ev[1], 0));
            hipLaunchKernelGGL(k_consensus_fast, dim3(cf_grid), dim3(256), 0, s, b, p, w);
        } else {
            hipLaunchKernelGGL(k_score2, dim3(sc2_grid), dim3(256), 0, s, b, p, w);
            hipLaunchKernelGGL(k_deep_prepare, dim3(1024), dim3(256), 0, s, b, p, w);
            hipLaunchKernelGGL(k_consensus_fast, dim3(cf_grid), dim3(256), 0, s, b, p, w);
        }
        hipLaunchKernelGGL(k_vote_deep, dim3(1024), dim3(DV_T), 0, s, b, p, w);
        LAUNCH_EV(k_consensus_slow, dim3(512), dim3(256), s, e->ev[EV_CONSENSUS], (const SlowArgs *)e->slow_args.p);
        CANARY("EV_CONSENSUS");
        hipLaunchKernelGGL(k_group_tail, dim3(cdiv(NG, 256)), dim3(256), 0, s, b, p, w, NG);
        if (!p.disable_duplex) {
            const unsigned nbc = cdiv(C, SCAN_TILE);
// ... 193 lines not shown
    HIPCHK(e->dp_depth.ensure((size_t)words * 8 + 64)); HIPCHK(e->dp_bed.ensure((size_t)nreg * 16 + 64));
    HIPCHK(hipMemsetAsync(e->dp_depth.p, 0, (size_t)words * 8, s)); HIPCHK(hipMemsetAsync(e->dp_bed.p, 0, (size_t)nreg * 16 + 16, s));
    DepthCtx c; c.bin_off = e->dp_binoff.as<int64_t>(); c.n_targets = nt; c.step = step; c.reg_off = e->dp_regoff.as<int32_t>();
    c.r_start = e->dp_rs.as<int32_t>(); c.r_end = e->dp_re.as<int32_t>(); c.r_pmax = e->dp_pmax.as<int32_t>(); c.contig_sorted = e->dp_sorted.as<uint8_t>();
    long long *pay = e->dp_depth.as<long long>();
    unsigned long long *dpre = (unsigned long long *)pay + 2 * GCE_STATS_WORDS, *dpost = dpre + nbins, *bpre = e->dp_bed.as<unsigned long long>(), *bpost = bpre + nreg;
    const uint64_t n = (uint64_t)e->n_pre, no = (uint64_t)e->n_out;
    if (n) hipLaunchKernelGGL(k_depth, dim3(cdiv(n, DP_T * DP_RPT)), dim3(DP_T), 0, s, e->dev_batch.core, (const uint32_t *)nullptr, n, c, dpre, bpre);
    if (no) hipLaunchKernelGGL(k_depth, dim3(cdiv(no, DP_T * DP_RPT)), dim3(DP_T), 0, s, e->dev_batch.core, (const uint32_t *)e->o_src.p, no, c, dpost, bpost);
    const int fin = std::max(2 * GCE_STATS_WORDS, (int)n_regions);
    hipLaunchKernelGGL(k_payload_finish, dim3(cdiv(fin, 256)), dim3(256), 0, s, (const StreamInfo *)e->si.p, (const int32_t *)e->dp_where.p, n_regions, (const unsigned long long *)e->dp_bed.p, nreg, pay, nbins);
    HIPCHK(hipGetLastError());
    HIPCHK(hipStreamSynchronize(s));
    layout->stats_words = 2 * GCE_STATS_WORDS; layout->n_targets = nt; layout->n_bins = nbins; layout->n_regions = n_regions; layout->total_words = words; layout->bin_off = e->h_binoff.data();
    e->payload_words = words;
    *payload = (const int64_t *)pay;
    return GCE_OK;
}

int gce_stats_payload_read(gce_engine *e, const int64_t *payload, int64_t n_words, int64_t *host) {
    if (!e || !payload || !host || n_words < 0) return GCE_ERR_INVALID;
    (void)hipSetDevice(e->prm.device);
    if (n_words) HIPCHK(hipMemcpyAsync(host, payload, (size_t)n_words * 8, hipMemcpyDeviceToHost, e->stream));
    HIPCHK(hipStreamSynchronize(e->stream));
    return GCE_OK;
}

int gce_depth_stats(gce_engine *e, int32_t step, int32_t n_regions, const int32_t *r_tid, const int32_t *r_start, const int32_t *r_end, gce_depth *out) {
    if (!e || !out) return GCE_ERR_INVALID;
    const int64_t *pay = nullptr; gce_payload_layout lay;
    int rc = gce_stats_payload_device(e, step, n_regions, r_tid, r_start, r_end, &pay, &lay);
    if (rc != GCE_OK) return rc;
    hipStream_t s = e->stream;
    const int64_t nbins = lay.n_bins;
    e->h_depth_pre.resize(nbins); e->h_depth_post.resize(nbins); e->h_bed_pre.assign(n_regions, 0); e->h_bed_post.assign(n_regions, 0);
    const int64_t *d0 = pay + lay.stats_words;
    if (nbins) { HIPCHK(hipMemcpyAsync(e->h_depth_pre.data(), d0, nbins * 8, hipMemcpyDeviceToHost, s)); HIPCHK(hipMemcpyAsync(e->h_depth_post.data(), d0 + nbins, nbins * 8, hipMemcpyDeviceToHost, s)); }
    if (n_regions) { HIPCHK(hipMemcpyAsync(e->h_bed_pre.data(), d0 + 2 * nbins, (size_t)n_regions * 8, hipMemcpyDeviceToHost, s)); HIPCHK(hipMemcpyAsync(e->h_bed_post.data(), d0 + 2 * nbins + n_regions, (size_t)n_regions * 8, hipMemcpyDeviceToHost, s)); }
    HIPCHK(hipStreamSynchronize(s));
    out->n_targets = lay.n_targets; out->bin_off = e->h_binoff.data(); out->pre_depth = e->h_depth_pre.data(); out->post_depth = e->h_depth_post.data();
    out->n_regions = n_regions; out->pre_bed = e->h_bed_pre.data(); out->post_bed = e->h_bed_post.data();
    return GCE_OK;
}

int gce_stats_device(gce_engine *e, const int64_t **pre_then_post) {
    if (!e || !pre_then_post || !e->processed || e->dev_error) return GCE_ERR_INVALID;
    *pre_then_post = (const int64_t *)e->si.as<StreamInfo>()->pre;
    return GCE_OK;
}

int gce_get_timing(gce_engine *e, gce_timing *out) {
    if (!e || !out) return GCE_ERR_INVALID;
    *out = e->timing;
    return GCE_OK;
}

int gce_get_vote_counters(gce_engine *e, int64_t out[4]) {
    if (!e || !out || !e->processed) return GCE_ERR_INVALID;
    out[0] = (int64_t)e->h_si.vote_rounds2; out[1] = (int64_t)e->h_si.vote_rounds2_unaligned;
    out[2] = (int64_t)(e->h_si.hand_on >> 32); out[3] = (int64_t)e->h_si.n_groups;
    return GCE_OK;
}

int gce_get_consensus_counters(gce_engine *e, int64_t out[5]) {
    if (!e || !out || !e->processed) return GCE_ERR_INVALID;
    out[0] = 2 * (int64_t)(e->h_si.n_groups ? e->h_si.n_live : 0) - (int64_t)(e->h_si.hand_on >> 32);
    out[1] = (int64_t)e->h_si.cs_fast; out[2] = (int64_t)e->h_si.cs_prep; out[3] = (int64_t)e->h_si.cs_deep; out[4] = (int64_t)e->h_si.cs_slow;
    return GCE_OK;
}

int gce_get_skipped_groups(gce_engine *e, int64_t out[2]) {
    if (!e || !out || !e->processed) return GCE_ERR_INVALID;
    out[0] = e->h_si.n_groups ? (int64_t)e->h_si.n_groups - (int64_t)e->h_si.n_live : 0;
    out[1] = e->h_si.n_groups ? (int64_t)(e->h_si.vote_weight / VB_W) + 1 : 0;
    return GCE_OK;
}

int gce_get_index_counters(gce_engine *e, int64_t out[4]) {
    if (!out) return GCE_ERR_INVALID;
    for (int k = 0; k < 4; k++) out[k] = e ? e->idx_ctr[k] : __atomic_load_n(&g_pass_idx_ctr[k], __ATOMIC_RELAXED);
    return GCE_OK;
}

int gce_get_pairing_tiers(gce_engine *e, int64_t cap, uint8_t *tier, uint32_t *read, int64_t *n_clusters, int64_t counts[GCE_PAIR_TIERS]) {
    if (!e || !e->processed || e->dev_error || cap < 0) return GCE_ERR_INVALID;
    const int64_t C = (int64_t)e->h_si.n_clusters;
    if (n_clusters) *n_clusters = C;
    if (counts) for (int k = 0; k < GCE_PAIR_TIERS; k++) counts[k] = 0;
    if (C == 0) return GCE_OK;
    if (!e->cl_tier.p || e->cl_tier.cap < (size_t)C) return fail(e, GCE_ERR_INVALID, "no pairing ran in the last gce_process");
    (void)hipSetDevice(e->prm.device);
    std::vector<uint8_t> t((size_t)C);
    HIPCHK(hipMemcpy(t.data(), e->cl_tier.p, (size_t)C, hipMemcpyDeviceToHost));
    if (counts) for (int64_t c = 0; c < C; c++) { if (t[c] >= GCE_PAIR_TIERS) return fail(e, GCE_ERR_INVALID, "a cluster has no pairing tier"); counts[t[c]]++; }
    const int64_t m = C < cap ? C : cap;
    if (tier) memcpy(tier, t.data(), (size_t)m);
    if (read && m > 0) {
        std::vector<uint32_t> st((size_t)m), pl((size_t)(e->n > 0 ? e->n : 1));
        HIPCHK(hipMemcpy(st.data(), e->cl_start.p, (size_t)m * 4, hipMemcpyDeviceToHost));
        HIPCHK(hipMemcpy(pl.data(), e->gpl.p, pl.size() * 4, hipMemcpyDeviceToHost));
        for (int64_t c = 0; c < m; c++) read[c] = (t[c] == GCE_PAIR_TIER_NEVER || st[c] >= pl.size()) ? 0xFFFFFFFFu : pl[st[c]];
    }
    return GCE_OK;
}

}

#include "gce_plan.hpp"
#include "gce_bamdev.hpp"
#include "gce_passes.hpp"
#include "gce_bai.hpp"
#include "gce_samdev.hpp"
#include "gce_samfmt.hpp"
#undef MCHK
#include "gce_sort.hpp"
#include "gce_calmd.hpp"
```

### gencore_amd/csrc/gce_device.hpp

```cpp
#pragma once
#include <hip/hip_runtime.h>
#include <stdint.h>
#include "../../include/gencore_amd.h"

#define GCE_WAVE 64
#define NONE32 0xFFFFFFFFu
#define EMPTY64 0xFFFFFFFFFFFFFFFFull

enum : uint32_t { THR_PROPER = 0, THR_UNPROPER = 1, THR_NEVER = 2, THR_RAW = 3 };
enum : uint8_t { TIER_NEVER = 0, TIER_SUB16 = 1, TIER_SUB32 = 2, TIER_FAST = 3, TIER_DEEP_LDS = 4, TIER_DEEP_DEVICE = 5, TIER_GENERIC = 6 };
enum : uint8_t { CLS_DROP = 0, CLS_CLUSTERED = 1, CLS_BYPASS = 2 };

struct DevBatch {
    int64_t n;
    const gce_core *core;
    const uint64_t *qname_off; const char *qname;
    const uint64_t *cigar_off; const uint32_t *cigar;
    const uint64_t *seq_off;   uint8_t *seq;
    const uint64_t *qual_off;  uint8_t *qual;
    const int32_t *nm; const uint8_t *nm_type;
    const uint64_t *mi_off; const char *mi;
    const uint64_t *tick;
};

struct DevParams {
    int32_t proper_thr, unproper_thr, duplex_mismatch_thr, cluster_size_req, base_score_req;
    int32_t high_q, moderate_q, low_q;
    int32_t s_high, s_moderate, s_low, s_bad;
    int32_t skip_low_complexity_thr, duplex_only, disable_duplex, period;
    int32_t score_bias, score_max;
    uint32_t q2s_lut;
    uint32_t thr_low4, thr_mod4, thr_high4;
    int32_t q2s_swar_ok;
    double score_percent_req;
    char prefix[32];
    int32_t prefix_len;
    int32_t n_targets;
    const uint32_t *target_len;
    const uint64_t *target_cum;
    int32_t key_bt, key_bl;
    int32_t nw_ok, nw_cb, nw_bd;
    int32_t vote_ok, vote_accept_by_qual, s_min_lb;
    int64_t tick_offset;
    int64_t tick_epoch0; int32_t tick_rem0;
    int32_t trailing_flush;
    int32_t n_ref;
    const uint8_t *const *ref_data;
    const int64_t *ref_len;
    const int64_t *ref_win;
};

#define GCE_PRE_SLOTS 64
struct StreamInfo {
    unsigned long long n_clustered;
    unsigned int first_unmapped;
    unsigned long long err_key;
    int n_events;
    int n_events_a;
    unsigned int n_slow;
    unsigned long long prof[32];
    unsigned int n_deep;
    unsigned long long hand_on;
    unsigned int n_slow_pair;
    unsigned int n_slow_pair2;
    unsigned int pair_next, pair_next2;
    unsigned int prep_next, deep_next;
    int lq_min, lq_max;
    unsigned long long n_clusters, n_groups, n_pairs, n_out;
    unsigned long long n_pairs_total;
    unsigned long long vote_weight;
    unsigned long long n_live;
    unsigned long long n_leaders;
    unsigned long long out_units;
    unsigned long long n_pf_items;
    unsigned long long n_pq_items;
    unsigned long long n_p16_items;
    unsigned long long vote_rounds2;
    unsigned long long vote_rounds2_unaligned;
    unsigned int n_raw;
    unsigned int cs_fast, cs_prep, cs_deep, cs_slow;
    long long pre[GCE_STATS_WORDS];
    long long post[GCE_STATS_WORDS];
    long long post_slot[GCE_PRE_SLOTS][8];
    long long pre_slot[GCE_PRE_SLOTS][8];
};

__device__ __forceinline__ void raise_error(StreamInfo *si, int code, uint32_t read) {
    atomicMin(&si->err_key, ((unsigned long long)read << 8) | (unsigned long long)((-code) & 0xFF));
}

__device__ __forceinline__ int lane_id() { return threadIdx.x & 63; }

__device__ __forceinline__ int cig_op(uint32_t w) { return (int)(w & 0xF); }
__device__ __forceinline__ int cig_len(uint32_t w) { return (int)(w >> 4); }
__device__ __forceinline__ int consumes_query(int op) { return (0x193 >> op) & 1; }
__device__ __forceinline__ int consumes_ref(int op) { return (0x18D >> op) & 1; }

struct __attribute__((aligned(16))) ReadDescP {
    uint32_t so_lo, qo_lo;
    uint32_t c0;
    uint32_t pos_fl;
    uint16_t lq, mo, ml, nc;
    int32_t tid;
    uint32_t hi;
};
static_assert(sizeof(ReadDescP) == 32, "ReadDescP must stay 32 bytes");
struct ReadDesc {
    uint64_t so, qo;
    uint32_t c0;
    int32_t pos, lq, isize;
    int32_t mo, ml;
    int32_t tid;
    uint16_t nc, lastm;
    int32_t rlen;
};
#define RLEN_WALK (-0x40000000)
__device__ __forceinline__ void store_desc(ReadDescP *base, uint64_t i, uint64_t so, uint64_t qo, uint32_t c0, int32_t pos, bool isize_nz, int lq, int mo, int ml, int nc, int32_t tid, uint32_t last_op) {
    union { ReadDescP d; uint4 q[2]; } u;
    u.d.so_lo = (uint32_t)so; u.d.qo_lo = (uint32_t)qo; const uint32_t lastm = cig_op(last_op) == 0 ? min((uint32_t)cig_len(last_op), 65535u) : 0u;
    u.d.hi = ((uint32_t)(so >> 32) & 0xFFu) | ((uint32_t)(qo >> 32) & 0xFFu) << 8 | lastm << 16;
    u.d.c0 = c0; u.d.pos_fl = (uint32_t)pos | (isize_nz ? 0x80000000u : 0u);
    u.d.lq = (uint16_t)lq; u.d.mo = (uint16_t)mo; u.d.ml = (uint16_t)ml; u.d.nc = (uint16_t)nc; u.d.tid = tid;
    uint4 *dst = reinterpret_cast<uint4 *>(base + i); dst[0] = u.q[0]; dst[1] = u.q[1];
}
__device__ __forceinline__ ReadDesc load_desc(const ReadDescP *base, uint32_t i) {
    union { ReadDescP d; uint4 q[2]; } u;
    const uint4 *src = reinterpret_cast<const uint4 *>(base + i);
    u.q[0] = src[0]; u.q[1] = src[1];
    ReadDesc r;
    r.so = (uint64_t)u.d.so_lo | (uint64_t)(u.d.hi & 0xFFu) << 32; r.qo = (uint64_t)u.d.qo_lo | (uint64_t)((u.d.hi >> 8) & 0xFFu) << 32;
    r.c0 = u.d.c0; r.pos = (int32_t)(u.d.pos_fl & 0x7FFFFFFFu); r.isize = (int32_t)(u.d.pos_fl >> 31);
    r.lq = u.d.lq; r.mo = u.d.mo; r.ml = u.d.ml; r.nc = u.d.nc; r.tid = u.d.tid; r.lastm = (uint16_t)(u.d.hi >> 16);
    r.rlen = u.d.nc == 1 ? (int32_t)(cig_len(u.d.c0) * consumes_ref(cig_op(u.d.c0))) : (u.d.nc == 0 ? 0 : RLEN_WALK);
    return r;
}


__device__ inline bool d_is_part_of(const uint32_t *part, int np, const uint32_t *whole, int nw, bool left) {
    if (nw < np) return false;
    for (int i = 0; i < np; i++) {
        uint32_t a = left ? part[i] : part[np - 1 - i];
        uint32_t b = left ? whole[i] : whole[nw - 1 - i];
        if (cig_op(a) != cig_op(b)) return false;
        int la = cig_len(a), lb = cig_len(b);
        if (la > lb) return false;
        if (la < lb && i != np - 1) {
            if (i != np - 2) return false;
            uint32_t nx = left ? part[i + 1] : part[np - 2 - i];
            if (cig_op(nx) != 5 ) return false;
        }
    }
    return true;
}

__device__ inline int d_ref_offset(const uint32_t *cig, int n, int qpos) {
    int ref = 0, query = 0;
    for (int i = 0; i < n; i++) {
        int op = cig_op(cig[i]), len = cig_len(cig[i]);
        int cq = consumes_query(op), cr = consumes_ref(op);
// ... 305 lines not shown
```

### gencore_amd/csrc/gce_kernels.hpp

```cpp
#pragma once
#include "gce_device.hpp"

#define CHUNK 256
#define WAVES_PER_BLOCK 4

struct __attribute__((aligned(16))) OutRec { uint32_t qname_src, mate; int16_t nm_new, fr, rr; uint16_t pad; };
static_assert(sizeof(OutRec) == 16, "OutRec must stay 16 bytes");

struct Work {
    uint64_t *uinfo;
    ReadDescP *rdesc;
    uint32_t *spatch;
    uint32_t *slot;
    int8_t *score;
    uint8_t *out_flag; OutRec *orec;
    uint32_t *nmx;
    uint32_t *out_index;
    struct LeadRec *lrec; struct LeadOut *lout;
    struct BlkHdr *bhdr; uint32_t *blk_base; int64_t n_sblk;
    int32_t *ev_tid, *ev_pos; uint32_t *ev_read; int max_events;
    struct TabEntry *tab; uint32_t *toff; uint64_t tsize; double tinv;
    uint32_t *cl_ikey, *cl_start, *cl_n, *cl_npairs, *cl_ngroups, *cl_gbase, *cl_nresult; uint8_t *cl_hasumi;
    uint8_t *cl_tier;
    uint32_t *members, *sorted, *pl, *pr, *pu, *pg, *gpl, *gpr, *grp_begin, *grp_n;
    uint64_t *k64;
    uint32_t *gl_cluster, *g_begin, *g_np;
    uint64_t *gw; uint4 *vlive; uint32_t *vb_start;
    uint32_t *slow_list;
    uint8_t *pf_flag; uint32_t *pf_list;
    uint8_t *pq_flag; uint32_t *pq_list;
    uint32_t *left_list;
    uint8_t *p16_flag; uint32_t *p16_list;
    void *deep_list;
    uint8_t *gen_flag; uint32_t *gen_list;
    uint32_t *score_list;
    uint32_t *rp_left, *rp_right, *rp_merge, *rp_rmerge; const char **rp_umi; uint16_t *rp_umilen; uint8_t *rp_state; int32_t *rp_supp;
    int32_t *rp_nm;
    uint32_t *rp_qsl, *rp_qsr;
    uint64_t *scan_part;
    StreamInfo *si;
};

#define UINFO_MAXLEN 32767
__device__ __forceinline__ uint64_t uinfo_pack(uint64_t off, bool from_mi, int l_qname, int len) {
    return (off & 0xFFFFFFFFFFull) | ((uint64_t)(from_mi ? 1 : 0) << 40) | ((uint64_t)(l_qname & 0xFF) << 41) | ((uint64_t)(len & 0x7FFF) << 49);
}
__device__ __forceinline__ const char *uinfo_ptr(const DevBatch &b, uint64_t v) { return (((v >> 40) & 1ull) ? b.mi : b.qname) + (v & 0xFFFFFFFFFFull); }
__device__ __forceinline__ int uinfo_len(uint64_t v) { return (int)(v >> 49); }
__device__ __forceinline__ bool uinfo_hm(uint64_t v) { return ((v >> 40) & 1ull) != 0; }
__device__ __forceinline__ int uinfo_lqname_pad(uint64_t v) { return ((int)((v >> 41) & 0xFFu) + 3) & ~3; }
__device__ __forceinline__ const char *d_umi_ptr(const DevBatch &b, const Work &w, uint64_t i) { return uinfo_ptr(b, w.uinfo[i]); }
__device__ __forceinline__ int d_umi_len(const Work &w, uint64_t i) { return uinfo_len(w.uinfo[i]); }
__device__ __forceinline__ bool d_umi_hm(const Work &w, uint64_t i) { return uinfo_hm(w.uinfo[i]); }
__device__ __forceinline__ int d_lqname(const Work &w, uint64_t i) { return (int)((w.uinfo[i] >> 41) & 0xFFu); }

enum : uint8_t { RP_PENDING = 0, RP_OUT_SSCS = 1, RP_OUT_DCS = 2, RP_DROPPED = 3, RP_CONSUMED = 4 };
#define NM_DEFER (-0x40000000)
#define NM_IS_DEFERRED(v) ((v) < -0x20000000)

#define WAVE_SYNC() do { __builtin_amdgcn_fence(__ATOMIC_SEQ_CST, "workgroup"); __builtin_amdgcn_wave_barrier(); } while (0)

__device__ __forceinline__ int rl32(int v, int l) { return __builtin_amdgcn_readlane(v, l); }
__device__ __forceinline__ uint64_t rl64(uint64_t v, int l) {
    uint32_t lo = (uint32_t)__builtin_amdgcn_readlane((int)(uint32_t)v, l), hi = (uint32_t)__builtin_amdgcn_readlane((int)(uint32_t)(v >> 32), l);
    return ((uint64_t)hi << 32) | lo;
}

__device__ __forceinline__ long long wave_sum64(long long v) {
    for (int o = 32; o > 0; o >>= 1) v += __shfl_xor(v, o);
    return v;
}

#include "gce_cluster.hpp"

__device__ __forceinline__ const char *d_qname(const DevBatch &b, uint32_t r) { return b.qname + b.qname_off[r]; }

typedef uint64_t u64_unaligned __attribute__((aligned(1)));
typedef uint32_t u32_unaligned __attribute__((aligned(1)));
__device__ __forceinline__ uint64_t d_bswap64(uint64_t x) { return __builtin_bswap64(x); }
template <int NW>
__device__ __forceinline__ void load_be_words(const char *s, int len, uint64_t (&wd)[NW]) {
#pragma unroll
    for (int k = 0; k < NW; k++) {
        uint64_t v = 0;
        int rem = len - 8 * k;
        if (rem > 0) {
            v = *(const u64_unaligned *)(s + 8 * k);
            if (rem < 8) v &= (1ull << (8 * rem)) - 1ull;
            v = d_bswap64(v);
        }
        wd[k] = v;
    }
}
template <int PHASE>
__device__ void pairing_generic(const DevBatch &b, const DevParams &p, const Work &w, uint32_t c, int lane, uint32_t ib0 = 0, uint32_t ibstep = 1) {
    const uint32_t start = w.cl_start[c], n = w.cl_n[c];
    uint32_t mode = d_thr_mode(w.cl_ikey[c], w.si, p);
    if (mode >= THR_NEVER) {
        if (PHASE == 2 && lane == 0) { w.cl_npairs[c] = 0; w.cl_ngroups[c] = 0; w.cl_hasumi[c] = 0; w.cl_tier[c] = TIER_NEVER; }
        return;
    }
    const int thr = mode == THR_PROPER ? p.proper_thr : p.unproper_thr;
    uint64_t *kw = w.k64 + (size_t)start * 3;
    if (PHASE == 0) {
        const char *n0 = d_qname(b, w.members[start]);
        int cp = 0x7FFFFFFF;
        for (uint32_t i = lane; i < n; i += 64) {
            const char *mq = d_qname(b, w.members[start + i]);
            int l = 0;
            while (n0[l] && n0[l] == mq[l]) l++;
            cp = min(cp, l);
        }
        cp = wave_min(cp);
        for (uint32_t i = lane; i < n; i += 64) {
            const uint32_t my = w.members[start + i];
// ... 261 lines not shown
        unsigned long long prev = act ? (EQ & LOW) : 0ull;
        const int rounds = wave_max(__popcll(prev));
        int plane = -1; uint32_t pv = 0;
        for (int r = 0; r < rounds; r++) {
            const bool has = prev != 0;
            const int src = has ? __ffsll((long long)prev) - 1 : lane;
            prev &= prev - 1;
            const uint32_t o = (uint32_t)__shfl((int)my, src);
            if (has && (plane < 0 || o > pv)) { pv = o; plane = src; }
        }
        if (rounds > 0) {
            const int src = plane < 0 ? lane : plane;
            const uint64_t q0 = (uint64_t)__shfl((long long)ruw[0], src), q1 = (uint64_t)__shfl((long long)ruw[1], src), q2 = (uint64_t)__shfl((long long)ruw[2], src);
            const int qul = __shfl(ul, src);
            if (plane >= 0 && qul != 0 && !(qul == ul && q0 == ruw[0] && q1 == ruw[1] && q2 == ruw[2])) raise_error(w.si, GCE_ERR_UMI_MISMATCH, my);
        }
    }
    const int any_umi = __any(act && last && ul > 0);
    const bool pact = lane < (int)npairs;
    uint32_t L = NONE32, R = NONE32, g_of = 0, ngroups = 1;
    {
        const int to_first = (first ? (int)pidx : 63) << 2, to_right = ((last && !first) ? (int)pidx : 63) << 2;
        L = (uint32_t)__builtin_amdgcn_ds_permute(to_first, first ? (int)(my + 1u) : 0) - 1u;
        R = (uint32_t)__builtin_amdgcn_ds_permute(to_right, (last && !first) ? (int)(my + 1u) : 0) - 1u;
        if (!pact) { L = NONE32; R = NONE32; }
    }
    if (any_umi) {
        uint64_t uw[3]; int ulen;
        {
            const int to_last = (last ? (int)pidx : 63) << 2;
#pragma unroll
            for (int k = 0; k < 3; k++) {
                const uint32_t lo = (uint32_t)__builtin_amdgcn_ds_permute(to_last, last ? (int)(uint32_t)ruw[k] : 0);
                const uint32_t hi = (uint32_t)__builtin_amdgcn_ds_permute(to_last, last ? (int)(uint32_t)(ruw[k] >> 32) : 0);
                uw[k] = pact ? (((uint64_t)hi << 32) | lo) : 0ull;
            }
            ulen = __builtin_amdgcn_ds_permute(to_last, last ? ul : 0);
            if (!pact) ulen = 0;
        }
        int cnt = 0, urank = 0;
        {
            const bool one_word = wave_max(ulen) <= 8;
            for (unsigned long long todo = __ballot(pact); todo;) {
                const int q = __ffsll((long long)todo) - 1;
                const uint64_t a0 = rl64(uw[0], q); const int al = rl32(ulen, q);
                bool eq, lt;
                if (one_word) { eq = a0 == uw[0] && al == ulen; lt = a0 != uw[0] ? a0 < uw[0] : al < ulen; }
                else {
                    const uint64_t a1 = rl64(uw[1], q), a2 = rl64(uw[2], q);
                    eq = a0 == uw[0] && a1 == uw[1] && a2 == uw[2] && al == ulen;
                    lt = a0 != uw[0] ? a0 < uw[0] : (a1 != uw[1] ? a1 < uw[1] : (a2 != uw[2] ? a2 < uw[2] : al < ulen));
                }
                const unsigned long long cls = __ballot(pact && eq);
                const int sz = __popcll(cls);
                if (pact && eq) cnt = sz;
                if (pact && lt) urank += sz;
                todo &= ~cls;
            }
        }
        g_of = NONE32; ngroups = 0;
        unsigned long long remaining = __ballot(pact);
        while (remaining) {
            int key = (pact && g_of == NONE32) ? (cnt * 64 + (63 - urank)) : -1;
            int best = wave_max(key);
            int tl = __ffsll((long long)__ballot(key == best)) - 1;
            uint64_t t0 = rl64(uw[0], tl), t1 = rl64(uw[1], tl), t2 = rl64(uw[2], tl);
            int diff = popc_nonzero_bytes(t0 ^ uw[0]) + popc_nonzero_bytes(t1 ^ uw[1]) + popc_nonzero_bytes(t2 ^ uw[2]);
            bool take = pact && g_of == NONE32 && diff <= thr;
            if (take) g_of = ngroups;
            remaining &= ~__ballot(take);
            ngroups++;
        }
    }
    uint32_t gbase = 0;
    for (uint32_t g = 0; g < ngroups; g++) {
        unsigned long long m = __ballot(pact && g_of == g);
        if (pact && g_of == g) { uint32_t d = start + gbase + lanes_below(m); w.gpl[d] = L; w.gpr[d] = R; }
        uint32_t run = __popcll(m);
        if (lane == 0) { w.grp_begin[start + g] = start + gbase; w.grp_n[start + g] = run; }
        gbase += run;
    }
    if (lane == 0) { const bool cross = d_key(b.core[w.members[start]], p).right < 0; w.cl_npairs[c] = npairs; w.cl_ngroups[c] = ngroups; w.cl_hasumi[c] = (uint8_t)((any_umi ? 1 : 0) | (cross ? 2 : 0)); w.cl_tier[c] = TIER_FAST; }
}
__global__ __launch_bounds__(256) void k_pairing_fast(DevBatch b, DevParams p, Work w, uint32_t n_clusters, const uint32_t *list) {
    const int lane = lane_id();
    const uint32_t total = list ? (uint32_t)w.si->n_pf_items : n_clusters, stride = gridDim.x * WAVES_PER_BLOCK;
    for (uint32_t idx = blockIdx.x * WAVES_PER_BLOCK + (threadIdx.x >> 6); idx < total; idx += stride) {
        pairing_fast_cluster(b, p, w, list ? list[idx] : idx, lane);
        WAVE_SYNC();
    }
}

__device__ __forceinline__ bool d_group_skipped(const DevParams &p, uint8_t cflags, uint32_t cl_groups, uint32_t np) {
    if (np != 1u || p.skip_low_complexity_thr < 1 || !(p.duplex_only || p.cluster_size_req > 1)) return false;
    return !(cflags & 1) || p.disable_duplex || cl_groups < 2u;
}

__global__ void k_group_fill(DevParams p, Work w, uint32_t n_clusters, uint32_t deep_weight, uint32_t min_weight) {
    uint32_t c = blockIdx.x * blockDim.x + threadIdx.x;
    if (c >= n_clusters) return;
    uint32_t g0 = w.cl_gbase[c], ng = w.cl_ngroups[c];
    const uint32_t cs = w.cl_start[c];
    const uint8_t cflags = ng ? w.cl_hasumi[c] : (uint8_t)0;
    for (uint32_t g = 0; g < ng; g++) {
        const uint32_t np = w.grp_n[cs + g], begin = w.grp_begin[cs + g];
        w.gl_cluster[g0 + g] = c; w.g_begin[g0 + g] = begin; w.g_np[g0 + g] = np;
        const uint64_t wt = np > 32u ? (uint64_t)deep_weight : (uint64_t)(np < min_weight ? min_weight : np);
        w.gw[g0 + g] = d_group_skipped(p, cflags, ng, np) ? 0ull : (wt | (1ull << 32));
    }
}
__global__ __launch_bounds__(256) void k_u32_apply(const uint32_t *in, uint32_t *out, uint64_t n, const uint64_t *part) {
    __shared__ uint64_t s_w[4];
    __shared__ uint64_t s_carry;
    const int lane = lane_id(), wv = threadIdx.x >> 6;
    if (threadIdx.x == 0) s_carry = part[blockIdx.x];
    __syncthreads();
    uint64_t base = (uint64_t)blockIdx.x * SCAN_TILE;
    for (int k = 0; k < SCAN_TILE / 256; k++) {
        uint64_t h = base + k * 256 + threadIdx.x;
        uint64_t v = tab_elem(in, h, n), x = v;
        for (int o = 1; o < 64; o <<= 1) { uint64_t t = (uint64_t)__shfl_up((long long)x, o); if (lane >= o) x += t; }
        if (lane == 63) s_w[wv] = x;
        __syncthreads();
        uint64_t woff = 0;
        for (int q = 0; q < wv; q++) woff += s_w[q];
        uint64_t carry = s_carry;
        if (h < n) out[h] = (uint32_t)(carry + woff + x - v);
        __syncthreads();
        if (threadIdx.x == 255) s_carry = carry + woff + x;
        __syncthreads();
    }
}

#define SC2_MAXU 1280
__global__ __launch_bounds__(256) void k_score2(DevBatch b, DevParams p, Work w) {
    __shared__ uint8_t s_map[WAVES_PER_BLOCK][SC2_MAXU];
    const int lane = lane_id(), wv = threadIdx.x >> 6;
    const uint32_t n_list = (uint32_t)w.si->hand_on;
    for (uint32_t base = (blockIdx.x * WAVES_PER_BLOCK + wv) * 64u; base < n_list; base += gridDim.x * WAVES_PER_BLOCK * 64u) {
    const uint32_t li = base + (uint32_t)lane;
    uint32_t L = NONE32, R = NONE32;
    if (li < n_list) { const uint32_t slot = w.score_list[li]; L = w.gpl[slot]; if (L != NONE32) R = w.gpr[slot]; }
    int lstart = 0, rstart = 0, cmp = 0;
    uint64_t lso = 0, rso = 0, lqo = 0, rqo = 0;
    if (L != NONE32) {
        if (R == NONE32) w.spatch[L] = GCE_PATCH_CONST;
        else {
            const ReadDesc lk = load_desc(w.rdesc, L), rk = load_desc(w.rdesc, R);
            if (!(lk.ml > 0 && rk.ml > 0)) { w.spatch[L] = GCE_PATCH_CONST; w.spatch[R] = GCE_PATCH_CONST; }
            else {
                const int dis = rk.pos - lk.pos;
                if (dis >= 0) { lstart = lk.mo + dis; rstart = rk.mo; cmp = min(lk.ml - dis, rk.ml); }
                else { lstart = lk.mo; rstart = rk.mo - dis; cmp = min(lk.ml, rk.ml + dis); }
                if (cmp > 0 && (lk.lq > 65535 || rk.lq > 65535)) { raise_error(w.si, GCE_ERR_INVALID, L); cmp = 0; }
                if (cmp > 0) {
                    w.spatch[L] = (uint32_t)lstart | ((uint32_t)cmp << 16); w.spatch[R] = (uint32_t)rstart | ((uint32_t)cmp << 16);
                    lso = lk.so; rso = rk.so; lqo = lk.qo; rqo = rk.qo;
                } else { cmp = 0; w.spatch[L] = 0u; w.spatch[R] = 0u; }
            }
        }
    }
    const int nu = (cmp + 7) >> 3;
    int pre = nu;
    for (int o = 1; o < 64; o <<= 1) { const int t = __shfl_up(pre, o); if (lane >= o) pre += t; }
    const int total = __shfl(pre, 63);
    pre -= nu;
    for (int ubase = 0; ubase < total; ubase += SC2_MAXU) {
        for (int k = 0; k < nu; k++) { const int u = pre + k - ubase; if (u >= 0 && u < SC2_MAXU) s_map[wv][u] = (uint8_t)lane; }
        WAVE_SYNC();
        const int lim = min(SC2_MAXU, total - ubase);
        for (int r0 = 0; r0 < lim; r0 += 64) {
// ... 1317 lines not shown
```

### gencore_amd/csrc/gce_pair2.hpp

```cpp
#pragma once

template <int SUB> __device__ __forceinline__ int sub_max(int v) {
    v = row_max16(v);
    if (SUB == 32) { const int t = __shfl_xor(v, 16); v = t > v ? t : v; }
    return v;
}
template <int SUB> __device__ __forceinline__ uint32_t sub_ballot(bool pr, int hb) {
    const unsigned long long m = __ballot(pr);
    return (uint32_t)(m >> hb) & (SUB == 32 ? 0xFFFFFFFFu : ((1u << (SUB & 31)) - 1u));
}
__device__ __forceinline__ uint64_t shfl64(uint64_t v, int src) { return (uint64_t)__shfl((long long)v, src); }

__device__ __forceinline__ int pair_class(uint32_t n) { return n <= 16u ? 0 : (n <= 32u ? 1 : 2); }
__global__ __launch_bounds__(256) void k_pair_class_reduce(const uint32_t *cl_n, uint32_t n_clusters, uint64_t *part) {
    __shared__ uint64_t s[4];
    const uint64_t base = (uint64_t)blockIdx.x * SCAN_TILE;
    uint64_t v = 0;
    for (int k = 0; k < SCAN_TILE / 256; k++) {
        const uint64_t i = base + k * 256 + threadIdx.x;
        if (i < n_clusters) { const int c = pair_class(cl_n[i]); v += c == 0 ? (1ull << 32) : (c == 1 ? 1ull : 0ull); }
    }
    v = (uint64_t)wave_sum64((long long)v);
    if (lane_id() == 0) s[threadIdx.x >> 6] = v;
    __syncthreads();
    if (threadIdx.x == 0) part[blockIdx.x] = s[0] + s[1] + s[2] + s[3];
}
__global__ __launch_bounds__(256) void k_pair_class_apply(const uint32_t *cl_n, uint32_t n_clusters, const uint64_t *part, uint32_t *l16, uint32_t *l32, uint32_t *l64, StreamInfo *si) {
    __shared__ uint32_t s_w[4][2];
    __shared__ uint32_t s_c0, s_c1;
    const int lane = lane_id(), wv = threadIdx.x >> 6;
    const uint64_t base = (uint64_t)blockIdx.x * SCAN_TILE;
    if (threadIdx.x == 0) { s_c0 = (uint32_t)(part[blockIdx.x] >> 32); s_c1 = (uint32_t)part[blockIdx.x]; }
    if (blockIdx.x == 0 && threadIdx.x == 0) si->n_pf_items = (unsigned long long)n_clusters - si->n_p16_items - si->n_pq_items;
    __syncthreads();
    for (int k = 0; k < SCAN_TILE / 256; k++) {
        const uint64_t i = base + k * 256 + threadIdx.x;
        const int c = i < n_clusters ? pair_class(cl_n[i]) : -1;
        const unsigned long long m0 = __ballot(c == 0), m1 = __ballot(c == 1);
        if (lane == 0) { s_w[wv][0] = (uint32_t)__popcll(m0); s_w[wv][1] = (uint32_t)__popcll(m1); }
        __syncthreads();
        uint32_t o0 = s_c0, o1 = s_c1, t0 = 0, t1 = 0;
        for (int q = 0; q < 4; q++) { if (q < wv) { o0 += s_w[q][0]; o1 += s_w[q][1]; } t0 += s_w[q][0]; t1 += s_w[q][1]; }
        const uint32_t r0 = o0 + (uint32_t)lanes_below(m0), r1 = o1 + (uint32_t)lanes_below(m1);
        if (c == 0) l16[r0] = (uint32_t)i;
        else if (c == 1) l32[r1] = (uint32_t)i;
        else if (c == 2) l64[(uint32_t)i - r0 - r1] = (uint32_t)i;
        __syncthreads();
        if (threadIdx.x == 0) { s_c0 += t0; s_c1 += t1; }
        __syncthreads();
    }
}
#ifdef PS_STOP
#define PS_TICK(k, live_) do { if ((k) >= PS_STOP) { if ((uint32_t)(live_) == 0xDEADBEEFu) flag_out[0] = 1; return; } } while (0)
#else
#define PS_TICK(k, live_) do { } while (0)
#endif
template <int SUB>
__global__ __launch_bounds__(256) void k_pairing_sub(DevBatch b, DevParams p, Work w, uint32_t n_clusters, const uint32_t *list, const unsigned long long *list_n, uint8_t *flag_out, int direct) {
    constexpr int PER = 64 / SUB;
    const int lane = lane_id(), hl = lane & (SUB - 1), hb = lane & ~(SUB - 1);
    const uint32_t idx = (blockIdx.x * WAVES_PER_BLOCK + (threadIdx.x >> 6)) * PER + (uint32_t)(lane / SUB);
    const uint32_t total = list ? (uint32_t)*list_n : n_clusters;
    if ((blockIdx.x * WAVES_PER_BLOCK + (threadIdx.x >> 6)) * PER >= total) return;
    bool live = idx < total;
    const uint32_t c = live ? (list ? list[idx] : idx) : 0u;
    uint32_t start = 0, n = 0; int thr = 0;
    if (live) {
        start = w.cl_start[c]; n = w.cl_n[c];
        const uint32_t mode = d_thr_mode(w.cl_ikey[c], w.si, p);
        if (mode >= THR_NEVER) { if (hl == 0) { w.cl_npairs[c] = 0; w.cl_ngroups[c] = 0; w.cl_hasumi[c] = 0; w.cl_tier[c] = TIER_NEVER; } live = false; }
        thr = mode == THR_PROPER ? p.proper_thr : p.unproper_thr;
    }
    uint32_t my = NONE32; int nl = 0; const char *nm = nullptr; int ul = 0;
    const char *up = nullptr;
    if (live && n <= (uint32_t)SUB && hl < (int)n) {
        my = w.members[start + hl];
        const uint64_t ui_ = w.uinfo[my];
        nl = (int)((ui_ >> 41) & 0xFFu) - 1;
        nm = d_qname(b, my);
        ul = uinfo_len(ui_);
        up = uinfo_ptr(b, ui_);
    }
    const uint32_t toolong = sub_ballot<SUB>(nl > 64 || ul > 24, hb);
    if (live && (n > (uint32_t)SUB || toolong)) {
        if (hl == 0) { if (direct) w.left_list[atomicAdd(&w.si->n_slow_pair2, 1u)] = c; else flag_out[c] = 1; }
        live = false;
    }
    if (!__any(live)) return;
    PS_TICK(0, my ^ (uint32_t)nl ^ (uint32_t)ul ^ (uint32_t)(uintptr_t)nm ^ (uint32_t)(uintptr_t)up);
    const bool act = live && hl < (int)n;
    const int nwords = (wave_max_u(act ? nl : 0) + 7) >> 3;
    uint64_t nw[8];
#pragma unroll
    for (int k = 0; k < 8; k++) {
        uint64_t v = 0;
        if (k < nwords) {
            const int rem = (act ? nl : 0) - 8 * k;
            if (rem > 0) { v = *(const u64_unaligned *)(nm + 8 * k); if (rem < 8) v &= (1ull << (8 * rem)) - 1ull; v = d_bswap64(v); }
        }
        nw[k] = v;
    }
    uint64_t ruw[3];
    load_be_words<3>(act ? up : nullptr, act ? ul : 0, ruw);
    uint32_t h32 = 0x9E3779B9u;
#pragma unroll
    for (int k = 0; k < 8; k++) if (k < nwords) {
        const uint32_t lo = (uint32_t)nw[k], hi = (uint32_t)(nw[k] >> 32);
        h32 = (__builtin_rotateleft32(h32, 5) ^ lo) + hi;
        h32 = __builtin_rotateleft32(h32, 11) ^ (hi + 0x7F4A7C15u);
    }
    h32 ^= h32 >> 15;
    PS_TICK(1, h32 ^ (uint32_t)(nw[0] ^ nw[1] ^ nw[2] ^ nw[3] ^ nw[4] ^ nw[5] ^ nw[6] ^ nw[7]) ^ (uint32_t)(ruw[0] ^ ruw[1] ^ ruw[2]));
    const int nmax = wave_max_u(live ? (int)n : 0);
    uint32_t EQ = 0, LOW = 0;
    {
        uint32_t todo = sub_ballot<SUB>(act, hb);
        while (__any(todo != 0)) {
            const int j = todo ? __ffs((int)todo) - 1 : hl;
            const uint32_t oh = (uint32_t)__shfl((int)h32, hb + j);
            const bool same = act && todo != 0 && h32 == oh;
            const uint32_t cls = sub_ballot<SUB>(same, hb);
            if (same) EQ = cls;
            todo &= ~cls;
        }
    }
    EQ &= ~(1u << hl);
    {
        bool bad = false;
        const int rounds = wave_max_u(act ? __popc(EQ) : 0);
        uint32_t rest = act ? EQ : 0u;
        for (int r = 0; r < rounds; r++) {
            const bool has = rest != 0;
            const int sl = has ? __ffs((int)rest) - 1 : hl;
            rest &= rest - 1;
            const uint32_t oj = (uint32_t)__shfl((int)my, hb + sl);
            if (has && oj < my) LOW |= 1u << sl;
#pragma unroll
            for (int k = 0; k < 8; k++) if (k < nwords) { const uint64_t o = shfl64(nw[k], hb + sl); if (has && o != nw[k]) bad = true; }
        }
        const uint32_t badm = sub_ballot<SUB>(bad, hb);
        if (live && badm) { if (hl == 0) { if (direct) w.left_list[atomicAdd(&w.si->n_slow_pair2, 1u)] = c; else w.slow_list[atomicAdd(&w.si->n_slow_pair, 1u)] = c; } live = false; }
    }
    if (!__any(live)) return;
    PS_TICK(2, EQ ^ (LOW << 1));
    const bool act2 = act && live;
    const bool first = act2 && !(EQ & LOW), last = act2 && !(EQ & ~LOW);
    const uint32_t FIRST = sub_ballot<SUB>(first, hb);
    const uint32_t npairs = __popc(FIRST);
// ... 64 lines not shown
            if (plane >= 0 && qul != 0 && !same) raise_error(w.si, GCE_ERR_UMI_MISMATCH, my);
        }
    }
    const bool any_umi = sub_ballot<SUB>(act2 && last && ul > 0, hb) != 0;
    const bool pact = live && hl < (int)npairs;
    uint32_t L, R, g_of = 0, ngroups = live ? 1u : 0u;
    {
        const int to_first = (hb + (first ? (int)pidx : SUB - 1)) << 2, to_right = (hb + ((last && !first) ? (int)pidx : SUB - 1)) << 2;
        L = (uint32_t)__builtin_amdgcn_ds_permute(to_first, first ? (int)(my + 1u) : 0) - 1u;
        R = (uint32_t)__builtin_amdgcn_ds_permute(to_right, (last && !first) ? (int)(my + 1u) : 0) - 1u;
        if (!pact) { L = NONE32; R = NONE32; }
    }
    PS_TICK(4, L ^ (R << 1) ^ (uint32_t)any_umi);
    if (__any(any_umi)) {
        uint64_t uw[3]; int ulen;
        {
            const int to_last = (hb + (last ? (int)pidx : SUB - 1)) << 2;
#pragma unroll
            for (int k = 0; k < 3; k++) {
                const uint32_t lo = (uint32_t)__builtin_amdgcn_ds_permute(to_last, last ? (int)(uint32_t)ruw[k] : 0);
                const uint32_t hi = (uint32_t)__builtin_amdgcn_ds_permute(to_last, last ? (int)(uint32_t)(ruw[k] >> 32) : 0);
                uw[k] = pact ? (((uint64_t)hi << 32) | lo) : 0ull;
            }
            ulen = __builtin_amdgcn_ds_permute(to_last, last ? ul : 0);
            if (!pact) ulen = 0;
        }
        const bool grp = any_umi;
        int cnt = 0, urank = 0;
        const bool one_word = wave_max_u(ulen) <= 8;
        {
            uint32_t todo = sub_ballot<SUB>(pact, hb);
            if (!grp) todo = 0u;
            while (__any(todo != 0)) {
                const bool open = todo != 0;
                const int q = open ? __ffs((int)todo) - 1 : hl;
                const uint64_t a0 = shfl64(uw[0], hb + q);
                bool eq, lt;
                if (one_word) { eq = a0 == uw[0]; lt = a0 < uw[0]; }
                else {
                    const int al = __shfl(ulen, hb + q);
                    const uint64_t a1 = shfl64(uw[1], hb + q), a2 = shfl64(uw[2], hb + q);
                    eq = a0 == uw[0] && a1 == uw[1] && a2 == uw[2] && al == ulen;
                    lt = a0 != uw[0] ? a0 < uw[0] : (a1 != uw[1] ? a1 < uw[1] : (a2 != uw[2] ? a2 < uw[2] : al < ulen));
                }
                const uint32_t cls = sub_ballot<SUB>(open && pact && eq, hb);
                const int sz = __popc(cls);
                if (open && pact && eq) cnt = sz;
                if (open && pact && lt) urank += sz;
                todo &= ~cls;
            }
        }
        if (grp) { g_of = NONE32; ngroups = 0; }
        uint32_t remaining = grp ? sub_ballot<SUB>(pact, hb) : 0u;
        while (__any(remaining != 0)) {
            const bool open = remaining != 0;
            const int key = (open && pact && g_of == NONE32) ? (cnt * 64 + (63 - urank)) : -1;
            const int best = sub_max<SUB>(key);
            const uint32_t bm = sub_ballot<SUB>(key == best && key >= 0, hb);
            const int tl = hb + (bm ? __ffs((int)bm) - 1 : hl);
            const uint64_t t0 = shfl64(uw[0], tl);
            int diff = popc_nonzero_bytes(t0 ^ uw[0]);
            if (!one_word) { const uint64_t t1 = shfl64(uw[1], tl), t2 = shfl64(uw[2], tl); diff += popc_nonzero_bytes(t1 ^ uw[1]) + popc_nonzero_bytes(t2 ^ uw[2]); }
            const bool take = open && pact && g_of == NONE32 && diff <= thr;
            if (take) g_of = ngroups;
            remaining &= ~sub_ballot<SUB>(take, hb);
            if (open) ngroups++;
        }
    }
    PS_TICK(5, g_of ^ (ngroups << 8) ^ L ^ R);
    {
        uint32_t gbase = 0;
        const int gmax = wave_max_u((int)ngroups);
        for (int g = 0; g < gmax; g++) {
            const bool in = pact && g_of == (uint32_t)g;
            const uint32_t m = sub_ballot<SUB>(in, hb);
            if (in) { const uint32_t d = start + gbase + __popc(m & ((1u << hl) - 1u)); w.gpl[d] = L; w.gpr[d] = R; }
            const uint32_t run = __popc(m);
            if (live && hl == 0 && g < (int)ngroups) { w.grp_begin[start + g] = start + gbase; w.grp_n[start + g] = run; }
            gbase += run;
        }
    }
    if (live && hl == 0) {
        const bool cross = d_key(b.core[w.members[start]], p).right < 0;
        w.cl_npairs[c] = npairs; w.cl_ngroups[c] = ngroups; w.cl_hasumi[c] = (uint8_t)((any_umi ? 1 : 0) | (cross ? 2 : 0)); w.cl_tier[c] = SUB == 16 ? TIER_SUB16 : TIER_SUB32;
    }
}
```

### gencore_amd/engine.py

```python
import ctypes as C

import numpy as np

from . import capi
from .batch import table_from_rows
from .capi import GceError, GceResult, GceStats, GceTiming

_ROW_FIELDS = (("src", np.uint32), ("kind", np.uint8), ("qname_src", np.uint32), ("nm_new", np.int32), ("fr", np.int16),
               ("rr", np.int16), ("mate", np.uint32), ("seq_off", np.uint64), ("qual_off", np.uint64))


def _copy_out(ptr, dt, cnt):
    addr = C.cast(ptr, C.c_void_p).value
    if not addr or cnt <= 0:
        return np.zeros(0, dt)
    return np.frombuffer(C.string_at(addr, int(cnt) * np.dtype(dt).itemsize), dtype=dt).copy()


class Engine:
    def __init__(self, params=None, **overrides):
        self.lib = capi.load_library()
        self.params = params if params is not None else capi.default_params(**overrides)
        self._keep = []
        self._h = C.c_void_p()
# ... 11 lines not shown
            self.close()
        except Exception:
            pass

    def _check(self, rc):
        if rc != 0:
            raise GceError(rc, self.lib.gce_last_error(self._h).decode(errors="replace"))

    def set_reference(self, tid, nibbles, n_bases):
        ptr = nibbles if isinstance(nibbles, int) else np.ascontiguousarray(nibbles, np.uint8).ctypes.data
        self._check(self.lib.gce_set_reference(self._h, tid, ptr, n_bases))

    def set_reference_ascii(self, tid, bases):
        if isinstance(bases, str):
            bases = bases.encode()
        a = np.frombuffer(bases, np.uint8) if isinstance(bases, (bytes, bytearray)) else np.ascontiguousarray(bases, np.uint8)
        self._check(self.lib.gce_set_reference_ascii(self._h, tid, a.ctypes.data, int(a.size)))

    def set_reference_window(self, tid, contig_len, win_start, bases):
        if isinstance(bases, str):
            bases = bases.encode()
        a = np.frombuffer(bases, np.uint8) if isinstance(bases, (bytes, bytearray)) else np.ascontiguousarray(bases, np.uint8)
        self._check(self.lib.gce_set_reference_window(self._h, tid, int(contig_len), int(win_start), a.ctypes.data, int(a.size)))

    def set_flush_events(self, ev_tid, ev_pos):
        t, p = np.ascontiguousarray(ev_tid, np.int32), np.ascontiguousarray(ev_pos, np.int32)
        self._check(self.lib.gce_set_flush_events(self._h, int(t.size), t.ctypes.data, p.ctypes.data))

    def add_reads(self, batch):
        st = batch.as_struct()
        self._check(self.lib.gce_submit(self._h, C.byref(st)))

    def add_reads_device(self, st, keepalive=None):
        self._keep = [st, keepalive]
        self._check(self.lib.gce_submit_device(self._h, C.byref(st)))

    def finish(self):
        self._check(self.lib.gce_process(self._h))

    def reset(self):
        self._check(self.lib.gce_reset(self._h))

    def timing(self):
        t = GceTiming()
        self._check(self.lib.gce_get_timing(self._h, C.byref(t)))
        return t.as_dict()

    def vote_counters(self):
        v = (C.c_int64 * 4)()
        self._check(self.lib.gce_get_vote_counters(self._h, v))
        return dict(rounds2=v[0], rounds2_unaligned=v[1], handed_on_sides=v[2], groups=v[3])

    CONSENSUS_KERNELS = ("vote", "fast", "deep_prepare", "vote_deep", "slow")

    def consensus_counters(self):
        v = (C.c_int64 * len(self.CONSENSUS_KERNELS))()
        self._check(self.lib.gce_get_consensus_counters(self._h, v))
        return dict(zip(self.CONSENSUS_KERNELS, (int(x) for x in v)))

    def skipped_groups(self):
        return self._skipped()[0]

    def vote_batches(self):
        return self._skipped()[1]

    def _skipped(self):
        v = (C.c_int64 * 2)()
        self._check(self.lib.gce_get_skipped_groups(self._h, v))
        return int(v[0]), int(v[1])

    def index_counters(self):
        return index_counters(self._h)

    PAIR_TIERS = ("never", "sub16", "sub32", "fast", "deep_lds", "deep_device", "generic")

    def pairing_tiers(self):
        n = C.c_int64(0)
        cnt = (C.c_int64 * len(self.PAIR_TIERS))()
        self._check(self.lib.gce_get_pairing_tiers(self._h, 0, None, None, C.byref(n), cnt))
        tier, read = np.zeros(n.value, np.uint8), np.zeros(n.value, np.uint32)
        self._check(self.lib.gce_get_pairing_tiers(self._h, n.value, tier.ctypes.data, read.ctypes.data, C.byref(n), cnt))
        return tier, read, dict(zip(self.PAIR_TIERS, (int(x) for x in cnt)))

    def rows(self):
        r = GceResult()
        self._check(self.lib.gce_drain(self._h, C.byref(r)))
        n = int(r.n_out)

        def arr(ptr, dt, cnt):
            if cnt == 0 or not ptr:
                return np.zeros(0, dt)
            return _copy_out(ptr, dt, cnt)

        rows = {name: arr(getattr(r, name), dt, n) for name, dt in _ROW_FIELDS}
        rows["seq"] = arr(r.seq, np.uint8, int(r.seq_bytes))
        rows["qual"] = arr(r.qual, np.uint8, int(r.qual_bytes))
        pre, post = GceStats(), GceStats()
        C.memmove(C.byref(pre), C.byref(r.pre), C.sizeof(GceStats))
        C.memmove(C.byref(post), C.byref(r.post), C.sizeof(GceStats))
        return rows, pre, post

    def output(self, batch):
        rows, pre, post = self.rows()
        t = table_from_rows(batch, rows, pre, post)
        t.out_index = np.sort(rows["src"])
        return t

    def depth_stats(self, step, regions):
        from .capi import GceDepth
        reg = np.asarray([r[:3] for r in regions], np.int32).reshape(-1, 3)
        t, a, b = (np.ascontiguousarray(reg[:, k]) for k in range(3))
        d = GceDepth()
        self._check(self.lib.gce_depth_stats(self._h, int(step), len(reg), t.ctypes.data, a.ctypes.data, b.ctypes.data, C.byref(d)))
        nt = d.n_targets
        off = _copy_out(d.bin_off, np.int64, nt + 1)
        nb = int(off[-1])
        get = lambda ptr, n: _copy_out(ptr, np.int64, n) if n else np.zeros(0, np.int64)
        return off, get(d.pre_depth, nb), get(d.post_depth, nb), get(d.pre_bed, len(reg)), get(d.post_bed, len(reg))

    def run(self, batch, reference=None):
        for tid, (nib, ln) in enumerate(reference or []):
            if nib is not None:
                self.set_reference(tid, nib, ln)
        self.add_reads(batch)
        self.finish()
        return self.output(batch)


def index_counters(handle=None):
    lib = capi.load_library()
    v = (C.c_int64 * 4)()
    rc = lib.gce_get_index_counters(handle, v)
    if rc != 0:
        raise GceError(rc, "gce_get_index_counters")
    return dict(segments=v[0], flagged=v[1], rounds=v[2], serial=v[3])


def run_stream(batch, params, reference=None, events=None):
    e = Engine(params)
    try:
        if events is not None:
            e.set_flush_events(*events)
        return e.run(batch, reference)
    finally:
        e.close()
```

### include/gencore_amd.h

```cpp
#ifndef GENCORE_AMD_H
#define GENCORE_AMD_H

#include <stddef.h>
#include <stdint.h>

#ifdef __cplusplus
extern "C" {
#endif

#define GCE_ABI_VERSION 3
#define GCE_NONE 0xFFFFFFFFu
#define GCE_MAX_SUPPORTING_READS 100

typedef struct gce_engine gce_engine;

typedef enum gce_status {
    GCE_OK = 0,
    GCE_ERR_INVALID = -1,
    GCE_ERR_NO_DEVICE = -2,
    GCE_ERR_HIP = -3,
    GCE_ERR_OOM = -4,
    GCE_ERR_UNSORTED = -10,
    GCE_ERR_UMI_MISMATCH = -11,
    GCE_ERR_NM_MISSING = -12,
// ... 98 lines not shown
    const uint8_t  *qual;
    size_t          seq_bytes, qual_bytes;
    gce_stats       pre;
    gce_stats       post;
} gce_result;

typedef struct gce_timing {
    double total_ms;
    double describe_ms;
    double cluster_ms;
    double csr_ms;
    double pairing_ms;
    double score_ms;
    double consensus_ms;
    double finish_ms;
    double output_ms;
    int64_t n_clusters, n_groups, n_pairs;
    int64_t n_leaders;
} gce_timing;

void gce_params_default(gce_params *p);

void gce_detect_umi_prefix(const char *first_qname, char out_prefix[32]);

int gce_create(const gce_params *params, gce_engine **out);
void gce_destroy(gce_engine *e);

int gce_set_reference(gce_engine *e, int32_t tid, const uint8_t *nibbles, int64_t n_bases);
int gce_set_reference_ascii(gce_engine *e, int32_t tid, const char *bases, int64_t n_bases);
int gce_set_reference_window(gce_engine *e, int32_t tid, int64_t contig_len, int64_t win_start, const char *bases, int64_t n_bases);
void gce_pack_reference(const char *bases, int64_t n_bases, uint8_t *nibbles_out);

int gce_set_flush_events(gce_engine *e, int32_t n_events, const int32_t *ev_tid, const int32_t *ev_pos);

int gce_submit(gce_engine *e, const gce_batch *batch);
int gce_submit_device(gce_engine *e, const gce_batch *batch);

int gce_process(gce_engine *e);

int gce_drain(gce_engine *e, gce_result *out);
int gce_result_device(gce_engine *e, gce_result *out);

int gce_reserve(gce_engine *e, int64_t n_reads, size_t qname_bytes, size_t cigar_words, size_t seq_bytes, size_t qual_bytes);
int gce_submit_async(gce_engine *e, const gce_batch *batch, int32_t *ticket);
int gce_submit_wait(gce_engine *e, int32_t ticket);

typedef struct gce_depth {
    int32_t        n_targets;
    const int64_t *bin_off;
    const int64_t *pre_depth;
    const int64_t *post_depth;
    int32_t        n_regions;
    const int64_t *pre_bed;
    const int64_t *post_bed;
} gce_depth;
int gce_depth_stats(gce_engine *e, int32_t coverage_step, int32_t n_regions, const int32_t *region_tid, const int32_t *region_start,
                    const int32_t *region_end, gce_depth *out);

typedef struct gce_payload_layout {
    int32_t stats_words;
    int32_t n_targets;
    int64_t n_bins;
    int32_t n_regions;
    int64_t total_words;
    const int64_t *bin_off;
} gce_payload_layout;
int gce_stats_payload_device(gce_engine *e, int32_t coverage_step, int32_t n_regions, const int32_t *region_tid, const int32_t *region_start,
                             const int32_t *region_end, const int64_t **payload, gce_payload_layout *layout);

int gce_get_timing(gce_engine *e, gce_timing *out);
int gce_get_vote_counters(gce_engine *e, int64_t out[4]);
int gce_get_consensus_counters(gce_engine *e, int64_t out[5]);
int gce_get_skipped_groups(gce_engine *e, int64_t out[2]);
int gce_get_index_counters(gce_engine *e, int64_t out[4]);
enum { GCE_PAIR_TIER_NEVER = 0,
       GCE_PAIR_TIER_SUB16 = 1,
       GCE_PAIR_TIER_SUB32 = 2,
       GCE_PAIR_TIER_FAST = 3,
       GCE_PAIR_TIER_DEEP_LDS = 4,
       GCE_PAIR_TIER_DEEP_DEVICE = 5,
       GCE_PAIR_TIER_GENERIC = 6,
       GCE_PAIR_TIERS = 7 };
int gce_get_pairing_tiers(gce_engine *e, int64_t cap, uint8_t *tier, uint32_t *read, int64_t *n_clusters, int64_t counts[GCE_PAIR_TIERS]);
int gce_stats_device(gce_engine *e, const int64_t **pre_then_post);

int gce_stream_context(int32_t device, const gce_core *core, int64_t n_reads, int32_t flush_period, uint64_t *tick_out,
                       int32_t *n_events, int32_t **ev_tid, int32_t **ev_pos);
int gce_plan_shards(int32_t device, const gce_core *core, int64_t n_reads, int32_t world, int32_t mode, int32_t *shard_out);
void gce_free(void *p);
int gce_reset(gce_engine *e);

const char *gce_last_error(const gce_engine *e);
const char *gce_status_message(int status);
int gce_abi_version(void);

typedef struct gce_bam gce_bam;
typedef struct gce_fasta gce_fasta;

typedef struct gce_bam_info {
    int32_t             n_targets;
    const uint32_t     *target_len;
    const char *const  *target_name;
    const char         *text;
    int64_t             l_text;
    int64_t             n_records;
    uint64_t            qname_bytes, cigar_words, seq_bytes, qual_bytes, mi_bytes;
    double              read_s, inflate_s, index_s;
} gce_bam_info;

int gce_bam_open(const char *path, int threads, gce_bam **out);
void gce_bam_close(gce_bam *f);
const char *gce_bam_error(const gce_bam *f);
int gce_bam_get_info(const gce_bam *f, gce_bam_info *out);
int gce_bam_chunk(gce_bam *f, int64_t first, int64_t count, int slot, gce_batch *out);
int gce_bam_write(const char *path, const gce_bam *in, const gce_result *res, int threads, int level);

int gce_bam_from_batch(const char *path, const gce_batch *batch, int32_t n_targets, const uint32_t *target_len,
                       const char *const *target_name, const char *text, int threads, int level);

int gce_sam_to_bam(const char *sam_path, const char *bam_path, int threads, int level, char err[256]);
int gce_bam_to_sam(const char *bam_path, const char *sam_path, int threads, char err[256]);

int gce_fasta_load(const char *path, int threads, gce_fasta **out);
int gce_fasta_get(const gce_fasta *fa, int32_t *n_contigs, const char *const **ids, const char *const **bases, const int64_t **lengths);
void gce_fasta_free(gce_fasta *fa);

int gce_bed_load(const char *path, int32_t n_targets, const char *const *target_name, int32_t *n_regions, int32_t **tid, int32_t **start,
                 int32_t **end, char ***name);
void gce_bed_free(int32_t n_regions, int32_t *tid, int32_t *start, int32_t *end, char **name);

typedef struct gce_bam_run {
    int64_t n_reads, n_out;
    double  open_s;
    double  read_s, inflate_s, index_s;
    double  submit_s;
    double  process_s;
    double  kernel_ms;
    double  drain_s, write_s, total_s;
    gce_stats pre, post;
    int64_t peak_rss_kb;
    int64_t rss_start_kb, rss_end_kb;
} gce_bam_run;
int gce_run_bam(const char *in_path, const char *out_path, const char *fasta_path, const gce_params *params, int threads,
                int64_t chunk_reads, int level, gce_bam_run *out, char err[256]);
int gce_run_bam_hostcodec(const char *in_path, const char *out_path, const char *fasta_path, const gce_params *params, int threads,
                          int64_t chunk_reads, int level, gce_bam_run *out, char err[256]);

int gce_raw_begin(gce_engine *e, size_t capacity_hint);
int gce_raw_push(gce_engine *e, const void *host, size_t bytes, int32_t *ticket);
int gce_raw_push_bgzf(gce_engine *e, const void *comp, size_t comp_bytes, int32_t n_members, const uint64_t *coff, const uint32_t *csize, const uint32_t *usize, int32_t *ticket);
int gce_bgzf_inflate(int32_t device, const void *comp, size_t comp_bytes, int32_t n_members, const uint64_t *coff, const uint32_t *csize, const uint32_t *usize, void *out, int32_t *first_bad);
int gce_raw_finish(gce_engine *e, uint64_t records_begin, int32_t n_ref, int64_t *n_records);
int gce_raw_build_output(gce_engine *e, uint64_t *body_bytes, int64_t *n_out);
int gce_raw_read_output_async(gce_engine *e, uint64_t offset, void *host, size_t bytes, int32_t *ticket);
int gce_raw_deflate_output(gce_engine *e, uint64_t *comp_bytes);
int gce_raw_read_deflated_async(gce_engine *e, uint64_t offset, void *host, size_t bytes, int32_t *ticket);
int gce_bgzf_deflate(int32_t device, const void *in, size_t n, uint32_t block_bytes, void *out, size_t out_cap, size_t *out_bytes);
int gce_raw_deflate_output_codes(gce_engine *e, int32_t codes, uint64_t *comp_bytes);
int gce_bgzf_deflate_codes(int32_t device, const void *in, size_t n, uint32_t block_bytes, int32_t codes, void *out, size_t out_cap, size_t *out_bytes);
int gce_host_alloc(size_t bytes, void **out);
void gce_host_free(void *p);

int gce_run_bam_sharded(const char *in_path, const char *out_path, const char *fasta_path, const gce_params *params, int32_t n_shards,
                        const int32_t *devices, int32_t plan_mode, int threads, int level, gce_bam_run *out, char err[256]);
int gce_run_bam_sharded_hostcodec(const char *in_path, const char *out_path, const char *fasta_path, const gce_params *params, int32_t n_shards,
                                  const int32_t *devices, int32_t plan_mode, int threads, int level, gce_bam_run *out, char err[256]);
// ... 93 lines not shown
```

Baseline: 1.931 billion.

## Add a 4-lane pairing tier and unify class lists into one partitioned array

Adds a fourth size class so clusters with at most four reads are paired by k_pairing_sub<4>, which packs 16 clusters per wave using DPP reductions instead of 16-lane subgroups. The per-class compaction is rewritten to scan four 16-bit counts per word into a single partitioned list with offsets kept in StreamInfo. The apply kernel now uses per-wave ballots instead of block-wide barriers per tile. The aim is to stop idle lanes in the many tiny clusters and to cut sync overhead in classification, at the cost of an extra launch and more tier code.

New measurement: 1.950 billion, median of 6. 1.01x the previous value.

```diff
diff --git a/gencore_amd/capi.py b/gencore_amd/capi.py
--- a/gencore_amd/capi.py
+++ b/gencore_amd/capi.py
@@ -93,7 +93,7 @@
 EXPORTED_SYMBOLS = [
     "gce_params_default", "gce_detect_umi_prefix", "gce_create", "gce_destroy", "gce_set_reference", "gce_set_reference_ascii", "gce_set_reference_window",
     "gce_pack_reference", "gce_set_flush_events", "gce_submit", "gce_submit_device", "gce_process", "gce_drain", "gce_result_device",
-    "gce_get_timing", "gce_get_vote_counters", "gce_get_consensus_counters", "gce_get_skipped_groups", "gce_get_index_counters", "gce_get_pairing_tiers", "gce_reset", "gce_last_error", "gce_status_message", "gce_abi_version",
+    "gce_get_timing", "gce_get_vote_counters", "gce_get_consensus_counters", "gce_get_skipped_groups", "gce_get_index_counters", "gce_get_pairing_tiers", "gce_get_pairing_classes", "gce_reset", "gce_last_error", "gce_status_message", "gce_abi_version",
     "gce_reserve", "gce_submit_async", "gce_submit_wait",
     "gce_bam_open", "gce_bam_close", "gce_bam_error", "gce_bam_get_info", "gce_bam_chunk", "gce_bam_write", "gce_bam_from_batch", "gce_sam_to_bam", "gce_bam_to_sam",
     "gce_fasta_load", "gce_fasta_get", "gce_fasta_free", "gce_run_bam", "gce_run_bam_hostcodec", "gce_run_bam_sharded", "gce_run_bam_sharded_hostcodec", "gce_raw_deflate_output", "gce_raw_read_deflated_async", "gce_bgzf_deflate", "gce_raw_deflate_output_codes", "gce_bgzf_deflate_codes", "gce_raw_attach_mirror", "gce_raw_select_shard", "gce_raw_merge_outputs", "gce_raw_begin", "gce_raw_push", "gce_raw_push_bgzf", "gce_bgzf_inflate", "gce_raw_finish", "gce_raw_build_output", "gce_raw_read_output_async", "gce_host_alloc", "gce_host_free", "gce_depth_stats", "gce_stats_payload_device", "gce_stats_payload_sum", "gce_stats_payload_read", "gce_run_bam_depth", "gce_depth_run_free", "gce_stats_device", "gce_stream_context", "gce_plan_shards", "gce_free", "gce_bed_load", "gce_bed_free",
@@ -201,6 +201,7 @@
     lib.gce_get_skipped_groups.argtypes = [C.c_void_p, C.POINTER(C.c_int64)]
     lib.gce_get_index_counters.argtypes = [C.c_void_p, C.POINTER(C.c_int64)]
     lib.gce_get_pairing_tiers.argtypes = [C.c_void_p, C.c_int64, C.c_void_p, C.c_void_p, C.POINTER(C.c_int64), C.POINTER(C.c_int64)]
+    lib.gce_get_pairing_classes.argtypes = [C.c_void_p, C.POINTER(C.c_int64), C.c_int]
     lib.gce_stats_device.argtypes = [C.c_void_p, C.POINTER(C.c_void_p)]
     lib.gce_stream_context.argtypes = [C.c_int32, C.c_void_p, C.c_int64, C.c_int32, C.c_void_p, C.POINTER(C.c_int32), C.POINTER(C.POINTER(C.c_int32)), C.POINTER(C.POINTER(C.c_int32))]
     lib.gce_plan_shards.argtypes = [C.c_int32, C.c_void_p, C.c_int64, C.c_int32, C.c_int32, C.c_void_p]
diff --git a/gencore_amd/csrc/engine.hip b/gencore_amd/csrc/engine.hip
--- a/gencore_amd/csrc/engine.hip
+++ b/gencore_amd/csrc/engine.hip
@@ -95,7 +95,7 @@
     bool tab_clean = false; const void *tab_clean_ptr = nullptr; size_t tab_clean_cap = 0;
     DevBuf cl_ikey, cl_start, cl_n, cl_npairs, cl_ngroups, cl_gbase, cl_nresult, cl_hasumi, cl_tier;
     DevBuf members, sorted, pl, pr, pu, pg, gpl, gpr, grp_begin, grp_n, gl_cluster, g_begin, g_np;
-    DevBuf slow_args, deep_list, k64, slow_list, left_list, pf_flag, pf_list, pq_flag, pq_list, p16_flag, p16_list, pd_slab, gen_flag, gen_list, score_list, gw, vlive, vb_start, rp_left, rp_right, rp_merge, rp_rmerge, rp_umi, rp_umilen, rp_state, rp_supp, rp_nm, rp_qsl, rp_qsr, scan_part, si;
+    DevBuf slow_args, deep_list, k64, slow_list, left_list, pf_flag, pf_list, pq_flag, pq_list, cls_list, pd_slab, gen_flag, gen_list, score_list, gw, vlive, vb_start, rp_left, rp_right, rp_merge, rp_rmerge, rp_umi, rp_umilen, rp_state, rp_supp, rp_nm, rp_qsl, rp_qsr, scan_part, si;
     StreamInfo h_si{};
     void *si_pin = nullptr, *si_pin_dev = nullptr; unsigned long long si_seq = 0;
     gce_timing timing{};
@@ -178,7 +178,7 @@
     for (auto *b : all) b->release();
     for (DevBuf *b : {&e->z_comp, &e->z_dir, &e->z_err, &e->raw, &e->rw_tmp, &e->rw_ncig, &e->rw_nmpos, &e->rw_rsize, &e->rw_roff, &e->rw_body, &e->sf_text}) b->release();
     e->rw.release();
-    for (DevBuf *b : {&e->zo_slots, &e->zo_sizes, &e->zo_off, &e->zo_out, &e->p16_flag, &e->p16_list}) b->release();
+    for (DevBuf *b : {&e->zo_slots, &e->zo_sizes, &e->zo_off, &e->zo_out, &e->cls_list}) b->release();
     for (DevBuf *b : {&e->sh_tickall, &e->sh_shard, &e->sh_flag, &e->sh_sel, &e->sh_core, &e->sh_qoff, &e->sh_coff, &e->sh_soff, &e->sh_loff, &e->sh_nm, &e->sh_nmt, &e->sh_mioff, &e->sh_tick, &e->sh_roff, &e->sh_nmpos, &e->sh_keys, &e->sh_stage}) b->release();
     for (DevBuf *b : {&e->dp_binoff, &e->dp_regoff, &e->dp_rs, &e->dp_re, &e->dp_pmax, &e->dp_sorted, &e->dp_depth, &e->dp_bed, &e->dp_where}) b->release();
     for (auto ev : e->up_events) (void)hipEventDestroy(ev);
@@ -741,7 +741,7 @@
     w.slow_list = e->slow_list.as<uint32_t>();
     ENS(deep_list, (n1 / 64 + 64) * 16); w.deep_list = e->deep_list.p;
     const unsigned nblk_N = cdiv(n1, SCAN_TILE);
-    ENS(scan_part, std::max<size_t>(2 * nsb1, (size_t)2 * nblk_N) * 8 + 16);     ENS(si, sizeof(StreamInfo));
+    ENS(scan_part, std::max<size_t>(2 * nsb1, (size_t)PAIR_NCLS * nblk_N) * 8 + 16);     ENS(si, sizeof(StreamInfo));
     w.uinfo = e->uinfo.as<uint64_t>(); w.rdesc = e->rdesc.as<ReadDescP>(); w.spatch = e->spatch.as<uint32_t>();
     w.slot = e->slot.as<uint32_t>(); w.score = e->score.as<int8_t>();
     w.out_flag = e->out_flag.as<uint8_t>(); w.nmx = e->nmx.as<uint32_t>(); w.orec = e->orec.as<OutRec>(); w.out_index = e->out_index.as<uint32_t>();
@@ -819,8 +819,8 @@
     bool si_behind_describe = false;
     if (C > 0 && e->dev_error == 0) {
         ENS(left_list, c1 * 4 + 64); w.left_list = e->left_list.as<uint32_t>();
-        ENS(pf_flag, c1 + 64); ENS(pf_list, c1 * 4); ENS(pq_flag, c1 + 64); ENS(pq_list, c1 * 4); ENS(p16_flag, c1 + 64); ENS(p16_list, c1 * 4);
-        w.pf_flag = e->pf_flag.as<uint8_t>(); w.pf_list = e->pf_list.as<uint32_t>(); w.pq_flag = e->pq_flag.as<uint8_t>(); w.pq_list = e->pq_list.as<uint32_t>(); w.p16_flag = e->p16_flag.as<uint8_t>(); w.p16_list = e->p16_list.as<uint32_t>();
+        ENS(pf_flag, c1 + 64); ENS(pf_list, c1 * 4); ENS(pq_flag, c1 + 64); ENS(pq_list, c1 * 4); ENS(cls_list, c1 * 4);
+        w.pf_flag = e->pf_flag.as<uint8_t>(); w.pf_list = e->pf_list.as<uint32_t>(); w.pq_flag = e->pq_flag.as<uint8_t>(); w.pq_list = e->pq_list.as<uint32_t>(); w.cls_list = e->cls_list.as<uint32_t>();
         const bool pair_classes = (double)N > 10.0 * (double)C;
         if (!pair_classes) fill_many(s, {FillSeg{e->pf_flag.p, c1, 0u, 0u}, FillSeg{e->pq_flag.p, c1, 0u, 0u}});
         const unsigned nbc = cdiv(C, SCAN_TILE);
@@ -833,9 +833,9 @@
         {
             hipEvent_t a_, b_, c_; (void)hipEventCreate(&a_); (void)hipEventCreate(&b_); (void)hipEventCreate(&c_);
             (void)hipEventRecord(a_, s);
-            hipLaunchKernelGGL(k_pairing_sub<16>, dim3(cdiv(C, 4 * WAVES_PER_BLOCK)), dim3(256), 0, s, b, p, w, C, (const uint32_t *)nullptr, (const unsigned long long *)nullptr, w.pq_flag, 0);
+            hipLaunchKernelGGL(k_pairing_sub<16>, dim3(cdiv(C, 4 * WAVES_PER_BLOCK)), dim3(256), 0, s, b, p, w, C, (const uint32_t *)nullptr, (const unsigned long long *)nullptr, (const unsigned long long *)nullptr, w.pq_flag, 0);
             (void)hipEventRecord(b_, s);
-            hipLaunchKernelGGL(k_pairing_sub<32>, dim3(cdiv(C, 2 * WAVES_PER_BLOCK)), dim3(256), 0, s, b, p, w, C, (const uint32_t *)nullptr, (const unsigned long long *)nullptr, w.pf_flag, 0);
+            hipLaunchKernelGGL(k_pairing_sub<32>, dim3(cdiv(C, 2 * WAVES_PER_BLOCK)), dim3(256), 0, s, b, p, w, C, (const uint32_t *)nullptr, (const unsigned long long *)nullptr, (const unsigned long long *)nullptr, w.pf_flag, 0);
             (void)hipEventRecord(c_, s); (void)hipEventSynchronize(c_);
             float m1 = 0, m2 = 0; (void)hipEventElapsedTime(&m1, a_, b_); (void)hipEventElapsedTime(&m2, b_, c_);
             fprintf(stderr, "k_pairing_sub up to tick %d: <16> %.3f ms, <32> over ALL clusters %.3f ms\n", PS_STOP, m1, m2);
@@ -844,9 +844,10 @@
 #endif
         ENS(pd_slab, PD_BIG_BLOCKS * PD_SLAB);
         if (pair_classes) {
+            const unsigned long long *cb = w.si->pair_cls;
             hipLaunchKernelGGL(k_pair_class_reduce, dim3(nbc), dim3(256), 0, s, (const uint32_t *)w.cl_n, C, w.scan_part);
-            hipLaunchKernelGGL(k_scan_partials, dim3(1), dim3(1024), 0, s, w.scan_part, (uint64_t)nbc, &w.si->n_p16_items, &w.si->n_pq_items);
-            hipLaunchKernelGGL(k_pair_class_apply, dim3(nbc), dim3(256), 0, s, (const uint32_t *)w.cl_n, C, (const uint64_t *)w.scan_part, w.p16_list, w.pq_list, w.pf_list, w.si);
+            hipLaunchKernelGGL(k_scan_partials, dim3(1), dim3(1024), 0, s, w.scan_part, (uint64_t)PAIR_NCLS * nbc, &w.si->n_pq_items , (unsigned long long *)nullptr);
+            hipLaunchKernelGGL(k_pair_class_apply, dim3(nbc), dim3(256), 0, s, (const uint32_t *)w.cl_n, C, (const uint64_t *)w.scan_part, w.cls_list, w.si);
             static const bool tiers_aux = getenv("GCE_NO_AUX_STREAM") == nullptr;
             hipStream_t s2 = s;
             if (tiers_aux) {
@@ -855,18 +856,19 @@
                 HIPCHK(hipEventRecord(e->aux_ev[0], s));
                 HIPCHK(hipStreamWaitEvent(s2, e->aux_ev[0], 0));
             }
-            hipLaunchKernelGGL(k_pairing_fast, dim3(2048), dim3(256), 0, s2, b, p, w, C, (const uint32_t *)w.pf_list);
+            hipLaunchKernelGGL(k_pairing_fast, dim3(2048), dim3(256), 0, s2, b, p, w, C, (const uint32_t *)w.cls_list, cb + PAIR_CLS_FAST, cb + PAIR_CLS_FAST + 1);
             hipLaunchKernelGGL(k_pairing_deep<false>, dim3(256), dim3(PD_T), 0, s2, b, p, w, (uint8_t *)nullptr);
             if (tiers_aux) HIPCHK(hipEventRecord(e->aux_ev[1], s2));
-            hipLaunchKernelGGL(k_pairing_sub<16>, dim3(cdiv(C, 4 * WAVES_PER_BLOCK)), dim3(256), 0, s, b, p, w, C, (const uint32_t *)w.p16_list, (const unsigned long long *)&w.si->n_p16_items, w.pq_flag, 1);
-            hipLaunchKernelGGL(k_pairing_sub<32>, dim3(cdiv(C, 2 * WAVES_PER_BLOCK)), dim3(256), 0, s, b, p, w, C, (const uint32_t *)w.pq_list, (const unsigned long long *)&w.si->n_pq_items, w.pf_flag, 1);
+            hipLaunchKernelGGL(k_pairing_sub<4>, dim3(cdiv(C, 16 * WAVES_PER_BLOCK)), dim3(256), 0, s, b, p, w, C, (const uint32_t *)w.cls_list, cb + PAIR_CLS_SUB4, cb + PAIR_CLS_SUB4 + 1, w.pq_flag, 1);
+            hipLaunchKernelGGL(k_pairing_sub<16>, dim3(cdiv(C, 4 * WAVES_PER_BLOCK)), dim3(256), 0, s, b, p, w, C, (const uint32_t *)w.cls_list, cb + PAIR_CLS_SUB16, cb + PAIR_CLS_SUB16 + 1, w.pq_flag, 1);
+            hipLaunchKernelGGL(k_pairing_sub<32>, dim3(cdiv(C, 2 * WAVES_PER_BLOCK)), dim3(256), 0, s, b, p, w, C, (const uint32_t *)w.cls_list, cb + PAIR_CLS_SUB32, cb + PAIR_CLS_SUB32 + 1, w.pf_flag, 1);
             if (tiers_aux) HIPCHK(hipStreamWaitEvent(s, e->aux_ev[1], 0));
         } else {
-            hipLaunchKernelGGL(k_pairing_sub<16>, dim3(cdiv(C, 4 * WAVES_PER_BLOCK)), dim3(256), 0, s, b, p, w, C, (const uint32_t *)nullptr, (const unsigned long long *)nullptr, w.pq_flag, 0);
+            hipLaunchKernelGGL(k_pairing_sub<16>, dim3(cdiv(C, 4 * WAVES_PER_BLOCK)), dim3(256), 0, s, b, p, w, C, (const uint32_t *)nullptr, (const unsigned long long *)nullptr, (const unsigned long long *)nullptr, w.pq_flag, 0);
             compact(w.pq_flag, w.pq_list, &w.si->n_pq_items);
-            hipLaunchKernelGGL(k_pairing_sub<32>, dim3(cdiv(C, 2 * WAVES_PER_BLOCK)), dim3(256), 0, s, b, p, w, C, (const uint32_t *)w.pq_list, (const unsigned long long *)&w.si->n_pq_items, w.pf_flag, 0);
+            hipLaunchKernelGGL(k_pairing_sub<32>, dim3(cdiv(C, 2 * WAVES_PER_BLOCK)), dim3(256), 0, s, b, p, w, C, (const uint32_t *)w.pq_list, (const unsigned long long *)nullptr, (const unsigned long long *)&w.si->n_pq_items, w.pf_flag, 0);
             compact(w.pf_flag, w.pf_list, &w.si->n_pf_items);
-            hipLaunchKernelGGL(k_pairing_fast, dim3(2048), dim3(256), 0, s, b, p, w, C, (const uint32_t *)w.pf_list);
+            hipLaunchKernelGGL(k_pairing_fast, dim3(2048), dim3(256), 0, s, b, p, w, C, (const uint32_t *)w.pf_list, (const unsigned long long *)nullptr, (const unsigned long long *)&w.si->n_pf_items);
             hipLaunchKernelGGL(k_pairing_deep<false>, dim3(256), dim3(PD_T), 0, s, b, p, w, (uint8_t *)nullptr);
         }
         hipLaunchKernelGGL(k_pairing_deep<true>, dim3(PD_BIG_BLOCKS), dim3(PD_T), 0, s, b, p, w, e->pd_slab.as<uint8_t>());
@@ -1226,6 +1228,13 @@
     return GCE_OK;
 }
 
+int gce_get_pairing_classes(gce_engine *e, int64_t *out, int n) {
+    static_assert(GCE_PAIR_CLASSES == PAIR_NCLS, "the header's class count");
+    if (!e || !out || n < 0 || !e->processed) return GCE_ERR_INVALID;
+    for (int k = 0; k < n; k++) out[k] = k < PAIR_NCLS ? (int64_t)(e->h_si.pair_cls[k + 1] - e->h_si.pair_cls[k]) : 0;
+    return GCE_OK;
+}
+
 int gce_get_pairing_tiers(gce_engine *e, int64_t cap, uint8_t *tier, uint32_t *read, int64_t *n_clusters, int64_t counts[GCE_PAIR_TIERS]) {
     if (!e || !e->processed || e->dev_error || cap < 0) return GCE_ERR_INVALID;
     const int64_t C = (int64_t)e->h_si.n_clusters;
diff --git a/gencore_amd/csrc/gce_device.hpp b/gencore_amd/csrc/gce_device.hpp
--- a/gencore_amd/csrc/gce_device.hpp
+++ b/gencore_amd/csrc/gce_device.hpp
@@ -74,7 +74,7 @@
     unsigned long long out_units;
     unsigned long long n_pf_items;
     unsigned long long n_pq_items;
-    unsigned long long n_p16_items;
+    unsigned long long pair_cls[5];
     unsigned long long vote_rounds2;
     unsigned long long vote_rounds2_unaligned;
     unsigned int n_raw;
diff --git a/gencore_amd/csrc/gce_kernels.hpp b/gencore_amd/csrc/gce_kernels.hpp
--- a/gencore_amd/csrc/gce_kernels.hpp
+++ b/gencore_amd/csrc/gce_kernels.hpp
@@ -30,7 +30,7 @@
     uint8_t *pf_flag; uint32_t *pf_list;
     uint8_t *pq_flag; uint32_t *pq_list;
     uint32_t *left_list;
-    uint8_t *p16_flag; uint32_t *p16_list;
+    uint32_t *cls_list;
     void *deep_list;
     uint8_t *gen_flag; uint32_t *gen_list;
     uint32_t *score_list;
@@ -458,11 +458,12 @@
     }
     if (lane == 0) { const bool cross = d_key(b.core[w.members[start]], p).right < 0; w.cl_npairs[c] = npairs; w.cl_ngroups[c] = ngroups; w.cl_hasumi[c] = (uint8_t)((any_umi ? 1 : 0) | (cross ? 2 : 0)); w.cl_tier[c] = TIER_FAST; }
 }
-__global__ __launch_bounds__(256) void k_pairing_fast(DevBatch b, DevParams p, Work w, uint32_t n_clusters, const uint32_t *list) {
+__global__ __launch_bounds__(256) void k_pairing_fast(DevBatch b, DevParams p, Work w, uint32_t n_clusters, const uint32_t *list, const unsigned long long *list_lo, const unsigned long long *list_hi) {
     const int lane = lane_id();
-    const uint32_t total = list ? (uint32_t)w.si->n_pf_items : n_clusters, stride = gridDim.x * WAVES_PER_BLOCK;
+    const uint32_t lo = (list && list_lo) ? (uint32_t)*list_lo : 0u;
+    const uint32_t total = list ? (uint32_t)*list_hi - lo : n_clusters, stride = gridDim.x * WAVES_PER_BLOCK;
     for (uint32_t idx = blockIdx.x * WAVES_PER_BLOCK + (threadIdx.x >> 6); idx < total; idx += stride) {
-        pairing_fast_cluster(b, p, w, list ? list[idx] : idx, lane);
+        pairing_fast_cluster(b, p, w, list ? list[lo + idx] : idx, lane);
         WAVE_SYNC();
     }
 }
diff --git a/gencore_amd/csrc/gce_pair2.hpp b/gencore_amd/csrc/gce_pair2.hpp
--- a/gencore_amd/csrc/gce_pair2.hpp
+++ b/gencore_amd/csrc/gce_pair2.hpp
@@ -1,6 +1,13 @@
 #pragma once
 
 template <int SUB> __device__ __forceinline__ int sub_max(int v) {
+    static_assert(SUB == 4 || SUB == 8 || SUB == 16 || SUB == 32, "sub-group widths of k_pairing_sub");
+    if (SUB <= 8) {
+        v = max(v, dpp_move<0xB1>(v));
+        v = max(v, dpp_move<0x4E>(v));
+        if (SUB == 8) v = max(v, dpp_move<0x141>(v));
+        return v;
+    }
     v = row_max16(v);
     if (SUB == 32) { const int t = __shfl_xor(v, 16); v = t > v ? t : v; }
     return v;
@@ -11,43 +18,59 @@
 }
 __device__ __forceinline__ uint64_t shfl64(uint64_t v, int src) { return (uint64_t)__shfl((long long)v, src); }
 
-__device__ __forceinline__ int pair_class(uint32_t n) { return n <= 16u ? 0 : (n <= 32u ? 1 : 2); }
+#define PAIR_NCLS 4
+enum { PAIR_CLS_SUB4 = 0, PAIR_CLS_SUB16 = 1, PAIR_CLS_SUB32 = 2, PAIR_CLS_FAST = 3 };
+__device__ __forceinline__ int pair_class(uint32_t n) { return n <= 4u ? PAIR_CLS_SUB4 : (n <= 16u ? PAIR_CLS_SUB16 : (n <= 32u ? PAIR_CLS_SUB32 : PAIR_CLS_FAST)); }
+static_assert(SCAN_TILE < 65536 && PAIR_NCLS <= 4, "16-bit class counts, four to a word");
+__device__ __forceinline__ uint32_t pair_cls_get(uint64_t v, int c) { return (uint32_t)(v >> (16 * c)) & 0xFFFFu; }
+#define PAIR_CLS_WAVE (SCAN_TILE / 4)
 __global__ __launch_bounds__(256) void k_pair_class_reduce(const uint32_t *cl_n, uint32_t n_clusters, uint64_t *part) {
     __shared__ uint64_t s[4];
-    const uint64_t base = (uint64_t)blockIdx.x * SCAN_TILE;
+    const int lane = lane_id(), wv = threadIdx.x >> 6;
+    const uint64_t base = (uint64_t)blockIdx.x * SCAN_TILE + (uint64_t)wv * PAIR_CLS_WAVE;
     uint64_t v = 0;
-    for (int k = 0; k < SCAN_TILE / 256; k++) {
-        const uint64_t i = base + k * 256 + threadIdx.x;
-        if (i < n_clusters) { const int c = pair_class(cl_n[i]); v += c == 0 ? (1ull << 32) : (c == 1 ? 1ull : 0ull); }
+    for (int k = 0; k < PAIR_CLS_WAVE / 64; k++) {
+        const uint64_t i = base + k * 64 + lane;
+        if (i < n_clusters) v += 1ull << (16 * pair_class(cl_n[i]));
     }
     v = (uint64_t)wave_sum64((long long)v);
-    if (lane_id() == 0) s[threadIdx.x >> 6] = v;
+    if (lane == 0) s[wv] = v;
     __syncthreads();
-    if (threadIdx.x == 0) part[blockIdx.x] = s[0] + s[1] + s[2] + s[3];
-}
-__global__ __launch_bounds__(256) void k_pair_class_apply(const uint32_t *cl_n, uint32_t n_clusters, const uint64_t *part, uint32_t *l16, uint32_t *l32, uint32_t *l64, StreamInfo *si) {
-    __shared__ uint32_t s_w[4][2];
-    __shared__ uint32_t s_c0, s_c1;
+    if (threadIdx.x < PAIR_NCLS) part[(uint64_t)threadIdx.x * gridDim.x + blockIdx.x] = pair_cls_get(s[0] + s[1] + s[2] + s[3], (int)threadIdx.x);
+}
+__global__ __launch_bounds__(256) void k_pair_class_apply(const uint32_t *cl_n, uint32_t n_clusters, const uint64_t *part, uint32_t *list, StreamInfo *si) {
+    __shared__ uint64_t s[4];
     const int lane = lane_id(), wv = threadIdx.x >> 6;
-    const uint64_t base = (uint64_t)blockIdx.x * SCAN_TILE;
-    if (threadIdx.x == 0) { s_c0 = (uint32_t)(part[blockIdx.x] >> 32); s_c1 = (uint32_t)part[blockIdx.x]; }
-    if (blockIdx.x == 0 && threadIdx.x == 0) si->n_pf_items = (unsigned long long)n_clusters - si->n_p16_items - si->n_pq_items;
+    const uint64_t base = (uint64_t)blockIdx.x * SCAN_TILE + (uint64_t)wv * PAIR_CLS_WAVE;
+    if (blockIdx.x == 0 && threadIdx.x <= PAIR_NCLS) si->pair_cls[threadIdx.x] = threadIdx.x < PAIR_NCLS ? part[(uint64_t)threadIdx.x * gridDim.x] : (unsigned long long)n_clusters;
+    int cls[PAIR_CLS_WAVE / 64];
+    uint64_t v = 0;
+#pragma unroll
+    for (int k = 0; k < PAIR_CLS_WAVE / 64; k++) {
+        const uint64_t i = base + k * 64 + lane;
+        cls[k] = i < n_clusters ? pair_class(cl_n[i]) : -1;
+        if (cls[k] >= 0) v += 1ull << (16 * cls[k]);
+    }
+    v = (uint64_t)wave_sum64((long long)v);
+    if (lane == 0) s[wv] = v;
     __syncthreads();
-    for (int k = 0; k < SCAN_TILE / 256; k++) {
-        const uint64_t i = base + k * 256 + threadIdx.x;
-        const int c = i < n_clusters ? pair_class(cl_n[i]) : -1;
-        const unsigned long long m0 = __ballot(c == 0), m1 = __ballot(c == 1);
-        if (lane == 0) { s_w[wv][0] = (uint32_t)__popcll(m0); s_w[wv][1] = (uint32_t)__popcll(m1); }
-        __syncthreads();
-        uint32_t o0 = s_c0, o1 = s_c1, t0 = 0, t1 = 0;
-        for (int q = 0; q < 4; q++) { if (q < wv) { o0 += s_w[q][0]; o1 += s_w[q][1]; } t0 += s_w[q][0]; t1 += s_w[q][1]; }
-        const uint32_t r0 = o0 + (uint32_t)lanes_below(m0), r1 = o1 + (uint32_t)lanes_below(m1);
-        if (c == 0) l16[r0] = (uint32_t)i;
-        else if (c == 1) l32[r1] = (uint32_t)i;
-        else if (c == 2) l64[(uint32_t)i - r0 - r1] = (uint32_t)i;
-        __syncthreads();
-        if (threadIdx.x == 0) { s_c0 += t0; s_c1 += t1; }
-        __syncthreads();
+    uint32_t mine = 0;
+    if (lane < PAIR_NCLS) {
+        mine = (uint32_t)part[(uint64_t)lane * gridDim.x + blockIdx.x];
+        for (int q = 0; q < wv; q++) mine += pair_cls_get(s[q], lane);
+    }
+    uint32_t off[PAIR_NCLS];
+#pragma unroll
+    for (int q = 0; q < PAIR_NCLS; q++) off[q] = (uint32_t)__builtin_amdgcn_readlane((int)mine, q);
+#pragma unroll
+    for (int k = 0; k < PAIR_CLS_WAVE / 64; k++) {
+        const uint64_t i = base + k * 64 + lane;
+#pragma unroll
+        for (int q = 0; q < PAIR_NCLS; q++) {
+            const unsigned long long m = __ballot(cls[k] == q);
+            if (cls[k] == q) list[off[q] + (uint32_t)lanes_below(m)] = (uint32_t)i;
+            off[q] += (uint32_t)__popcll(m);
+        }
     }
 }
 #ifdef PS_STOP
@@ -56,14 +79,15 @@
 #define PS_TICK(k, live_) do { } while (0)
 #endif
 template <int SUB>
-__global__ __launch_bounds__(256) void k_pairing_sub(DevBatch b, DevParams p, Work w, uint32_t n_clusters, const uint32_t *list, const unsigned long long *list_n, uint8_t *flag_out, int direct) {
+__global__ __launch_bounds__(256) void k_pairing_sub(DevBatch b, DevParams p, Work w, uint32_t n_clusters, const uint32_t *list, const unsigned long long *list_lo, const unsigned long long *list_hi, uint8_t *flag_out, int direct) {
     constexpr int PER = 64 / SUB;
     const int lane = lane_id(), hl = lane & (SUB - 1), hb = lane & ~(SUB - 1);
     const uint32_t idx = (blockIdx.x * WAVES_PER_BLOCK + (threadIdx.x >> 6)) * PER + (uint32_t)(lane / SUB);
-    const uint32_t total = list ? (uint32_t)*list_n : n_clusters;
+    const uint32_t lo = (list && list_lo) ? (uint32_t)*list_lo : 0u;
+    const uint32_t total = list ? (uint32_t)*list_hi - lo : n_clusters;
     if ((blockIdx.x * WAVES_PER_BLOCK + (threadIdx.x >> 6)) * PER >= total) return;
     bool live = idx < total;
-    const uint32_t c = live ? (list ? list[idx] : idx) : 0u;
+    const uint32_t c = live ? (list ? list[lo + idx] : idx) : 0u;
     uint32_t start = 0, n = 0; int thr = 0;
     if (live) {
         start = w.cl_start[c]; n = w.cl_n[c];
@@ -294,6 +318,7 @@
     }
     if (live && hl == 0) {
         const bool cross = d_key(b.core[w.members[start]], p).right < 0;
-        w.cl_npairs[c] = npairs; w.cl_ngroups[c] = ngroups; w.cl_hasumi[c] = (uint8_t)((any_umi ? 1 : 0) | (cross ? 2 : 0)); w.cl_tier[c] = SUB == 16 ? TIER_SUB16 : TIER_SUB32;
-    }
-}
+        w.cl_npairs[c] = npairs; w.cl_ngroups[c] = ngroups; w.cl_hasumi[c] = (uint8_t)((any_umi ? 1 : 0) | (cross ? 2 : 0)); w.cl_tier[c] = SUB <= 16 ? TIER_SUB16 : TIER_SUB32;
+    }
+}
+template __global__ void k_pairing_sub<8>(DevBatch, DevParams, Work, uint32_t, const uint32_t *, const unsigned long long *, const unsigned long long *, uint8_t *, int);
diff --git a/gencore_amd/engine.py b/gencore_amd/engine.py
--- a/gencore_amd/engine.py
+++ b/gencore_amd/engine.py
@@ -117,6 +117,13 @@
         self._check(self.lib.gce_get_pairing_tiers(self._h, n.value, tier.ctypes.data, read.ctypes.data, C.byref(n), cnt))
         return tier, read, dict(zip(self.PAIR_TIERS, (int(x) for x in cnt)))
 
+    PAIR_CLASS_MAX_READS = (4, 16, 32, None)
+
+    def pairing_classes(self):
+        v = (C.c_int64 * len(self.PAIR_CLASS_MAX_READS))()
+        self._check(self.lib.gce_get_pairing_classes(self._h, v, len(v)))
+        return [int(x) for x in v]
+
     def rows(self):
         r = GceResult()
         self._check(self.lib.gce_drain(self._h, C.byref(r)))
diff --git a/include/gencore_amd.h b/include/gencore_amd.h
--- a/include/gencore_amd.h
+++ b/include/gencore_amd.h
@@ -204,6 +204,8 @@
        GCE_PAIR_TIER_GENERIC = 6,
        GCE_PAIR_TIERS = 7 };
 int gce_get_pairing_tiers(gce_engine *e, int64_t cap, uint8_t *tier, uint32_t *read, int64_t *n_clusters, int64_t counts[GCE_PAIR_TIERS]);
+#define GCE_PAIR_CLASSES 4
+int gce_get_pairing_classes(gce_engine *e, int64_t *out, int n);
 int gce_stats_device(gce_engine *e, const int64_t **pre_then_post);
 
 int gce_stream_context(int32_t device, const gce_core *core, int64_t n_reads, int32_t flush_period, uint64_t *tick_out,
```
